# Tongdongq/darwin-gpu

Measured on AMD Instinct MI355X. Metric: GACT GCUPS (DP cells/s) on ~10 kb PacBio-shape reads, higher is better.
Workload: dtype int16x2 (packed); 1 GPU; ecoli10x_self_overlap; tile_size=320, tile_overlap=120, scoring=+1/-1/-1/-1, reads=4642, bases=48503677, candidates=65766, tiles=2185214, parallelism=candidates dealt round-robin over 1 GPU(s), slots_in_flight=4, passes_in_this_process=127, arch=gfx950:sramecc+:xnack-

## Files before the change

darwin-gpu_amd/csrc/gact_coop.hpp:

```cpp
#pragma once

#include "gact_lin.hpp"

namespace gact {

constexpr int kCoopBanks = 2;
constexpr int kCoopJobs = (kBlockThreads / 64) * 8 * kCoopBanks;
static_assert(kCoopJobs == 64, "a walking wave serves every job of its block, one per lane");
constexpr int kCoopCacheStride = 36;

struct CoopJob {
    uint32_t ws_off;
    int R, Q;
    int k0;
    int v0;
    int band_lim;
    uint32_t where;
    int pad_;
};
struct CoopDone { int ref_steps, query_steps, dv, redo; };

template <class L> constexpr size_t coop_bank_words() { return (size_t)L::G::kMaxFlush * L::kWalkQuads * kWsRow * 4; }
template <class L> __host__ constexpr size_t coop_ws_words(int blocks) { return (size_t)blocks * (kBlockThreads / 64) * kCoopBanks * coop_bank_words<L>(); }

// ... 60 lines not shown
        const uint32_t rw = stage[seg + (rp >> 4)], qw = stage[seg + kSeg + (qp >> 4)];
        rcode = __builtin_amdgcn_ubfe(rw, ((uint32_t)rp & 15u) << 1, 2u);
        qcode = __builtin_amdgcn_ubfe(qw, ((uint32_t)qp & 15u) << 1, 2u);
    };
#ifdef GACT_STAMPS
    unsigned long long n_trips = 0, n_lane_trips = 0;
#endif
    while (__any(go)) {
        if (go) {
            tb_refill_oct<CW, QN, ROW>(ws_all, ws_off, scratch, l, c, k, rg);
            off0 = 4 * (-8 * rg.fbase[0] - 4 * rg.qbase0);
            off1 = 4 * (16 - 8 * rg.fbase[1] - 4 * (QN - 2));
            cur = fetch(l, c, k);
            bases();
        }
#pragma unroll 1
        for (int m = 0; m < 8; m++) {
            if (!__any(go)) break;
#ifdef GACT_STAMPS
            n_trips++; n_lane_trips += (unsigned long long)__builtin_popcountll(__ballot(go));
#endif
            if (go) {
                const bool diag = cur == kM;
                const int sub = rcode == qcode ? v_match : v_mism;
                v -= diag ? sub : v_gap;
                nis -= cur != kD;
                njs -= cur != kI;
                const int p = imax(p0 + njs, 0);
                l = (int)(__umul24((uint32_t)p, kMagic) >> 16);
                c = p + __mul24(l, -CW);
                k = imax(kA + l + nis, 0);
                if (m == 7) {
                    redo = redo | ((band_lim >= 0) & ((unsigned)(nis - njs + band_lim) > (unsigned)(2 * band_lim)));
                } else {
                    cur = fetch(l, c, k);
                    bases();
                }
                go = !((diag && v == 0) || nis <= nlim_i || njs <= nlim_j || redo);
            }
        }
    }
    if (active) {
        done[lane].ref_steps = -nis; done[lane].query_steps = -njs; done[lane].dv = v0 - v; done[lane].redo = redo ? 1 : 0;
        __builtin_amdgcn_fence(__ATOMIC_RELEASE, "workgroup");
        __hip_atomic_store(&jstate[lane], st0 + 2u, __ATOMIC_RELAXED, __HIP_MEMORY_SCOPE_WORKGROUP);
    }
#ifdef GACT_STAMPS
    {
        const unsigned long long n_jobs = (unsigned long long)__builtin_popcountll(__ballot(active));
        if (lane == 0) { atomicAdd(&g_coop_counts[0], 1ull); atomicAdd(&g_coop_counts[1], n_trips); atomicAdd(&g_coop_counts[2], n_lane_trips);
                         atomicAdd(&g_coop_counts[3], n_jobs); }
    }
#endif
}

template <class L, bool TWO_SETS = false>
__global__ __launch_bounds__(kBlockThreads, 3) void extend_coop_kernel(
    KParams kp, P16Consts kc, SeqSetDev refs, SeqSetDev qfwd, SeqSetDev qrc,
    int same_file, gact_overlap *__restrict__ out, ChainQueues cq,
    uint32_t *__restrict__ ws_all)
{
    using G = typename L::G;
    constexpr int LANES = L::kLanes;
    static_assert(LANES == kGroup && L::kWalkFmt == 3 && L::kEndAligned, "the split linear-gap layout");
    constexpr int kGroupsOfWave = 64 / LANES;
    constexpr int kGroupsPerBlock = (kBlockThreads / 64) * kGroupsOfWave;
    constexpr int kStageWords = StageGeom<L::kSlotsPerLane, LANES>::kWords;
    constexpr int kSeg = StageGeom<L::kSlotsPerLane, LANES>::kSeg;
    static_assert(((kGroupsPerBlock * kCoopBanks * kStageWords) >> 15) == 0, "stage index fits CoopJob::where");
    constexpr int kRefBytes = (G::kRefBytes + 15) & ~15;
    __shared__ __attribute__((aligned(16))) uint8_t lds[kGroupsPerBlock * kRefBytes];
    __shared__ ChainState chain_lds[kGroupsPerBlock][kCoopBanks][kSlots];
    __shared__ __attribute__((aligned(16))) uint32_t stage_lds[kGroupsPerBlock][kCoopBanks][kStageWords];
    __shared__ __attribute__((aligned(16))) CoopJob jobs[kCoopJobs];
    __shared__ CoopDone done[kCoopJobs];
    __shared__ uint32_t jstate[kCoopJobs];
    __shared__ __attribute__((aligned(16))) uint32_t cache_lds[kCoopJobs * kCoopCacheStride];
    __shared__ int bank_lds[kGroupsPerBlock][kCoopBanks][6];
    __shared__ uint32_t walk_lock;

    uint32_t *const lin_lut = LinLutLds<L::kLutWords>::get();
    for (int n = threadIdx.x; n < kCoopJobs; n += kBlockThreads) jstate[n] = 0;
    if (threadIdx.x == 0) walk_lock = 0;
    lin_lut_fill(lin_lut, kc, (int)threadIdx.x);
    __syncthreads();

    const int wave_in_block = threadIdx.x >> 6;
    WaveCtx w;
    {
        const int lane = threadIdx.x & 63;
        w.gl = lane & (LANES - 1);
        w.g = lane / LANES;
        w.slot = (blockIdx.x * (kBlockThreads / 64) + wave_in_block) * kGroupsOfWave + w.g;
        w.n_slots = gridDim.x * (kBlockThreads / 64) * kGroupsOfWave;
    }
    const int group_in_block = wave_in_block * kGroupsOfWave + w.g;
    uint8_t *ref8 = lds + group_in_block * kRefBytes;
    uint8_t *q8 = ref8;
    const uint16_t *ref16_lane = reinterpret_cast<const uint16_t *>(ref8) + (L::kRow0 - 1 - w.gl);
    uint32_t *ws_wave = ws_all + (size_t)(blockIdx.x * (kBlockThreads / 64) + wave_in_block) * (kCoopBanks * coop_bank_words<L>());
    const int job_base = (group_in_block * kSlots + (w.gl & 1)) * kCoopBanks;

    for (int b = 0; b < kCoopBanks; b++)
        if (w.gl < kSlots) { chain_lds[group_in_block][b][w.gl].phase = 2; chain_lds[group_in_block][b][w.gl].cand = -1; }
    if (w.gl == 0) {
        int *bt = &bank_lds[group_in_block][0][0];
        for (int n = 0; n < kCoopBanks * 6; n++) bt[n] = 0;
    }
    wave_sync();
    bool exhausted = false;
    int my_bucket = 0;
    int bucket_first = 0;
    if (cq.leave_longest > 0) {
        int acc = 0;
        while (bucket_first < kBuckets && (acc += cq.bucket_count[bucket_first]) <= cq.leave_longest) bucket_first++;
        if (bucket_first >= kBuckets) bucket_first = 0;
    }
    bool second_set = false;
    constexpr bool one_set = !TWO_SETS;
    int idle_polls = 0;
    int rank_turn = 0, rank_cached = 0;
    int bank = 0;
    __builtin_amdgcn_s_setprio(3);
#ifdef GACT_STAMPS
    unsigned long long stamp_acc[8] = {0, 0, 0, 0, 0, 0, 0, 0};
    const unsigned long long tl_start = __builtin_amdgcn_s_memrealtime();
    const unsigned long long tl_cyc0 = __builtin_amdgcn_s_memtime();
    unsigned long long tl_empty = 0;
#endif

    for (;;) {
        ChainState *st = chain_lds[group_in_block][bank];
        GACT_STAMP(t_w0);
        const int *bk = &bank_lds[group_in_block][bank][0];
        const uint32_t want = (uint32_t)__builtin_amdgcn_readfirstlane(bk[4]);
        if (want != 0) {
            const int sv_R[kSlots] = {bk[0], bk[2]}, sv_Q[kSlots] = {bk[1], bk[3]};
            const bool mine = w.gl < kSlots && ((w.gl & 1) ? sv_R[1] : sv_R[0]) > 0;
            const int my_job = job_base + bank;
            const unsigned long long wd0 = __builtin_amdgcn_s_memrealtime();
            for (;;) {
                const uint32_t s = mine ? __hip_atomic_load(&jstate[my_job], __ATOMIC_RELAXED, __HIP_MEMORY_SCOPE_WORKGROUP) : want;
                if (__all(s == want)) break;
                if (__any(mine && (s & 3u) == 1u)) {
                    uint32_t got = 1;
                    if ((threadIdx.x & 63) == 0) got = atomicCAS(&walk_lock, 0u, 1u);
                    got = (uint32_t)__builtin_amdgcn_readfirstlane((int)got);
                    if (got == 0) {
                        __builtin_amdgcn_fence(__ATOMIC_ACQUIRE, "workgroup");
                        coop_walk_batch<L>(kp, ws_all, jobs, jstate, done, &stage_lds[0][0][0], cache_lds);
                        __builtin_amdgcn_fence(__ATOMIC_RELEASE, "workgroup");
                        if ((threadIdx.x & 63) == 0) __hip_atomic_store(&walk_lock, 0u, __ATOMIC_RELAXED, __HIP_MEMORY_SCOPE_WORKGROUP);
                        continue;
                    }
                }
                __builtin_amdgcn_s_sleep(4);
                if (__builtin_amdgcn_s_memrealtime() - wd0 > 200000000ull) {
                    if ((threadIdx.x & 63) == 0) atomicOr(cq.band_redos, 1 << 30);
                    break;
                }
            }
            __builtin_amdgcn_fence(__ATOMIC_ACQUIRE, "workgroup");
            int ref_steps = 0, query_steps = 0, nst = 0, redo = 0;
            ScoreWalk wk;
            wk.score = 0; wk.pend_gap = 0; wk.open_flag = 0; wk.have_left = 0; wk.left_first_gap = 0;
            if (mine) {
                const CoopDone d = done[my_job];
// ... 202 lines not shown
```

darwin-gpu_amd/csrc/gact_engine.hip:

```cpp
#include <hip/hip_runtime.h>
#include <rccl/rccl.h>

#include <cerrno>
#include <dlfcn.h>
#include <fcntl.h>
#include <unistd.h>

#include <algorithm>
#include <atomic>
#include <chrono>
#include <condition_variable>
#include <cstdarg>
#include <cstdio>
#include <cstring>
#include <deque>
#include <memory>
#include <mutex>
#include <string>
#include <thread>
#include <vector>

#include "gact_hip.h"
#include "gact_kernels.hpp"
#include "gact_chain_kernel.hpp"
// ... 279 lines not shown
    {"force_wide", "GACT_HIP_FORCE_WIDE", 'c', 'k', "the wide layout (32 lanes per tile pair) for every main launch"},
    {"no_wide", "GACT_HIP_NO_WIDE", 'c', 'k', "never the wide layout"},
    {"no_tagged", "GACT_HIP_NO_TAGGED", 'c', 'k', "explicit pointer comparisons instead of tagged scores"},
    {"no_lin", "GACT_HIP_NO_LIN", 'c', 'k', "the affine passes also for linear scorings (gact_lin.hpp off)"},
    {"no_aff", "GACT_HIP_NO_AFF", 'c', 'k', "round 1's tagged affine pass instead of the drifted one (gact_aff.hpp off)"},
    {"coop", "GACT_HIP_COOP", 'l', 'k', "the split linear-gap main launch with two banks of tiles per wave and cooperative, batched traceback walks (gact_coop.hpp): 1 always, 0 never, 2 / unset where throughput bounds the launch"},
    {"roles", "GACT_HIP_ROLES", 'l', 'k', "1: the split linear-gap main launch as DP waves + walker waves (gact_roles.hpp; default 0: measured no faster, DESIGN 3.13)"},
    {"no_routing", "GACT_HIP_NO_ROUTING", 'c', 'k', "a set with a non-ACGT byte moves the whole launch onto the raw-byte kernels"},
    {"no_side_lane", "GACT_HIP_NO_SIDE_LANE", 'c', 's', "routed raw-byte launches after the 2-bit ones instead of beside them"},
    {"band", "GACT_HIP_BAND", 'c', 'k', "width of the stored pointer band in columns (default 48; 0: the whole window)"},
    {"poison_ws", "GACT_HIP_POISON_WS", 'c', 'k', "<seed>: seeded garbage over the traceback workspace before every launch (tests)"},
    {"no_overlap", "GACT_HIP_NO_OVERLAP", 'c', 's', "seed launch, then one main launch, always; live: overlap_seed"},
    {"overlap_seed", nullptr, 'l', 's', "1 / 0: ordered, overlapped seeding of large runs on an idle engine"},
    {"shared_twelfths", "GACT_HIP_SHARED_TWELFTHS", 'l', 's', "<n>: a linear-gap main launch that shares the machine and has more chains than two thirds of the resident tile slots hold takes n twelfths of the resident blocks (default 6)"},
    {"lone_lane", "GACT_HIP_LONE_LANE", 'l', 's', "<n>: a run of half as many to as many chains as there are resident tile slots, alone on the machine, runs as one block per CU of two kinds: n wide blocks for its longest chains, split blocks with the look-ahead walker on the other CUs (-n: without it); 0 (default): all wide, two blocks per CU"},
    {"overlap_big", "GACT_HIP_OVERLAP_BIG", 'l', 's', "1 / 0 (default): ... also of runs of more than four chains per resident tile slot (seed launch A takes the longest eighth, B the rest beside main launch 1; +1.3 % on pacbio50mb alone)"},
    {"no_crit_lane", "GACT_HIP_NO_CRIT_LANE", 'c', 's', "no wide launch beside the split one for runs of 1-1.5 chains per tile slot"},
    {"crit_lane_always", "GACT_HIP_CRIT_LANE_ALWAYS", 'c', 's', "... also for runs of up to four chains per tile slot"},
    {"no_shared_hint", "GACT_HIP_NO_SHARED_HINT", 'c', 's', "a launch made while another slot runs may take the wide layout"},
    {"runs_in_flight", nullptr, 'l', 's', "1: the caller keeps several runs in flight (every launch takes the throughput layout)"},
    {"no_combine", "GACT_HIP_NO_COMBINE", 'c', 's', "runs of several threads are never merged into one launch; live: combine"},
    {"combine", nullptr, 'l', 's', "1 / 0: the call combiner"},
    {"combine_window_us", "GACT_HIP_COMBINE_US", 'l', 's', "how long a leader waits for the other feeder threads (default 1000)"},
    {"sdma_copies", "GACT_HIP_SDMA_COPIES", 'c', 's', "candidate lists and records through hipMemcpyAsync instead of a copy kernel"},
    {"dsoft_temp_cap", "GACT_HIP_DSOFT_TEMP_CAP", 'c', 'k', "initial size of the device filter's candidate staging area (tests: forces the regrow path)"},
    {"rccl_lib", "GACT_HIP_RCCL_LIB", 'c', 's', "<file>: the RCCL library gact_hip_comm_create loads"},
    {"path_budget_mb", "GACT_HIP_PATH_BUDGET_MB", 'c', 's', "<n>: MiB of column buffers a path run (gact_hip_candidates_paths) takes at most; larger selections run in chunks (default 1024)"},
    {"no_aff_seed", "GACT_HIP_NO_AFF_SEED", 'c', 'd', "round 1's packed seed pass for affine scorings"},
    {"lane_blocks", "GACT_HIP_LANE_BLOCKS", 'c', 'd', "<n>: blocks of the critical lane"},
    {"lane_small", "GACT_HIP_LANE_SMALL", 'c', 'd', "<f>: the lane also instead of the all-wide launch, for runs of at least f/2 chains per lane tile"},
    {"no_chain_prio", "GACT_HIP_NO_CHAIN_PRIO", 'c', 'd', "all DP passes at issue priority 0"},
    {"static_prio", "GACT_HIP_STATIC_PRIO", 'c', 'd', "fixed priority thresholds instead of the ranking against the longest running chain"},
    {"rank16", "GACT_HIP_RANK16", 'c', 'd', "the ranking's two thresholds in sixteenths, hi << 8 | mid (default 12, 8)"},
    {"team_when_shared", "GACT_HIP_TEAM_WHEN_SHARED", 'c', 'd', "look-ahead walker in split launches that share the machine"},
    {"wide_blocks_per_cu", "GACT_HIP_WIDE_BLOCKS_PER_CU", 'c', 'd', "<n>: resident blocks per CU of the wide launch"},
    {"band_quantum", "GACT_HIP_BAND_QUANTUM", 'c', 'd', "<1|4|8>: lanes store their band in aligned groups"},
    {"lin_blocks", "GACT_HIP_LIN_BLOCKS", 'c', 'd', "<n>: a smaller persistent grid for the one-wave-does-all split linear-gap launch"},
    {"role_blocks", "GACT_HIP_ROLE_BLOCKS", 'c', 'd', "<n>: a smaller persistent grid for the role launch"},
    {"trace", "GACT_HIP_TRACE", 'c', 'd', "every launch of a run named on stderr and waited for"},
    {"trace_upload", "GACT_HIP_TRACE_UPLOAD", 'c', 'd', "stamps inside candidates_upload / _fetch on stderr"},
};
static const char *opt_env(const char *name)
{
    for (const OptionDef &o : kOptions)
        if (!strcmp(o.name, name)) {
#ifndef GACT_EXPERIMENTS
            if (o.klass == 'd') return nullptr;
#endif
            return o.env ? getenv(o.env) : nullptr;
        }
    fprintf(stderr, "[gact_hip] internal: switch '%s' is not in the option table\n", name);
    abort();
}

struct RunReq {
    int slot, first, n, rc_from, same_file;
    int status = 0;
    bool launched = false;
    std::string err;
};
struct Combiner {
    std::mutex mu;
    std::condition_variable cv;
    std::vector<RunReq *> pending;
    bool leader = false;
    bool enabled = true;
    int window_us = 1000;
    int next_merge = 0;
    int n_merge = 0;
    long merged_launches = 0, merged_runs = 0, rejoins = 0;
    std::vector<std::shared_ptr<LaunchStats>> stats_pool;
};

struct gact_hip_engine {
    gact_hip_params params;
    gact::KParams kp{};
    int C = 20;
    int big_cb = 0;
    int big_blocks = 0;
    bool p16 = false;
    bool split = false;
    bool tagged = false;
    bool lin = false;
    bool aff = false;
    bool aff_seed = true;
    int wide = 0;
    int wide_blocks_per_cu = 0;
    bool crit_lane = true;
    int lane_blocks = 0;
    bool lane_small = false;
    int lane_small_factor = 3;
    bool crit_lane_always = false;
    bool kernel_copies = true;
    bool shared_hint = true;
    std::atomic<bool> caller_keeps_runs_in_flight{false};
    bool team_when_shared = false;
    bool overlap_seed = true;
    bool side_lane = true;
    bool route_other = true;
    bool chain_prio = true;
    bool static_prio = false;
    uint32_t poison = 0;
    int rank16 = (12 << 8) | 8;
    bool seed16 = false;
    int seed_grid_blocks = 0;
    int seed_lin_grid_blocks = 0;
    int lin_grid_blocks = 0;
    bool roles = false;
    int role_grid_blocks = 0;
    int shared_twelfths = 6;
    int lone_lane = 0;
    bool overlap_big = false;
    int coop = 0;
    int64_t path_budget = 1024ll << 20;
    int aff_grid_blocks = 0;
    int wide_lin_grid_blocks = 0;
    gact::P16Consts kc;
    hipDeviceProp_t prop;
    int grid_blocks = 0;
    int blocks_per_cu = 0;
    size_t ws_words_total = 0;
    SeqSet sets[GACT_NUM_SETS];
    std::vector<Slot> slots;
    int n_user = 0;
    Combiner cb;
    std::mutex upload_mu;
    int64_t sets_epoch = 0;
    DsoftState dsoft;
    std::mutex dsoft_mu;
    int64_t ref_epoch = 0;
    Pileup pileup;
};

namespace {

int set_device(gact_hip_engine *e)
{
    HIP_TRY(hipSetDevice(e->params.device_id));
    return 0;
}

int check_slot(gact_hip_engine *e, int slot)
{
    if (!e) return fail(GACT_HIP_EINVAL, "engine is NULL");
    if (slot < 0 || slot >= e->n_user)
        return fail(GACT_HIP_EINVAL, "slot %d out of range [0,%d)", slot, e->n_user);
    return 0;
}

void note_call(gact_hip_engine *e, int slot)
{
    if (!e->cb.enabled || e->n_user < 2) return;
    std::lock_guard<std::mutex> lk(e->cb.mu);
    Slot &sl = e->slots[slot];
    sl.last_thread = std::this_thread::get_id();
    sl.last_call = std::chrono::steady_clock::now();
}

constexpr int kMoreCount = 8 + 2 * gact::kBuckets + gact::kEpochs, kMorePop = kMoreCount + gact::kBuckets;
constexpr int kOrderHist = kMorePop + gact::kBuckets, kOrderCursor = kOrderHist + gact::kBuckets;
constexpr int kCounterInts = kOrderCursor + gact::kBuckets;

int poison_ws(gact_hip_engine *e, Slot &sl, uint32_t salt);

struct StreamPool {
    std::mutex mu;
// ... 238 lines not shown
    const Lane own = main_lane(e, sl);
    const int blocks = std::max(1, std::min((n + 3) / 4, e->big_blocks));
    auto k = e->big_cb == 16 ? gact::big_extend_kernel<16> : gact::big_extend_kernel<32>;
    hipLaunchKernelGGL(k, dim3(blocks), dim3(gact::kBlockThreads), 0, sl.stream, e->kp, rs.dev(true), qf.dev_or(true, rs),
                       qr.dev_or(true, rs), sl.cands.p, first, n, rc_from, same_file, sl.overlaps.p, queues(own, sl),
                       reinterpret_cast<uint8_t *>(sl.d_ws));
    HIP_TRY(hipGetLastError());
    return 0;
}

gact_policy::Caps policy_caps(const gact_hip_engine *e)
{
    gact_policy::Caps c;
    c.C = e->C; c.p16 = e->p16; c.seed16 = e->seed16; c.lin = e->lin; c.aff = e->aff; c.aff_seed = e->aff_seed; c.split = e->split; c.tagged = e->tagged;
    c.mismatch_below_extend = e->params.mismatch < e->params.gap_extend;
    c.shared_twelfths = e->shared_twelfths; c.lone_lane = e->lone_lane; c.overlap_big = e->overlap_big; c.roles = e->roles; c.coop = (e->lin && e->split && e->C == 20) ? e->coop : -1; c.overlap_seed = e->overlap_seed; c.crit_lane = e->crit_lane; c.crit_lane_always = e->crit_lane_always;
    c.lane_small = e->lane_small; c.lane_small_factor = e->lane_small_factor; c.lane_blocks = e->lane_blocks; c.team_when_shared = e->team_when_shared;
    c.wide = e->wide; c.wide_blocks_per_cu = e->wide_blocks_per_cu; c.cus = e->prop.multiProcessorCount;
    c.grid_blocks = e->grid_blocks; c.seed_grid_blocks = e->seed_grid_blocks; c.seed_lin_grid_blocks = e->seed_lin_grid_blocks;
    c.lin_grid_blocks = e->lin_grid_blocks; c.aff_grid_blocks = e->aff_grid_blocks; c.wide_lin_grid_blocks = e->wide_lin_grid_blocks;
    c.role_grid_blocks = e->role_grid_blocks; c.role_dp_waves = gact::kRoleDp;
    c.ws_words_per_tile = (size_t)e->kp.ws_words;
    c.role_ws_words_per_block = gact::role_ws_words<gact::SplitLayoutLin<7, 13>>(1);
    c.coop_ws_words_per_block = gact::coop_ws_words<gact::SplitLayoutLin<7, 13>>(1);
    return c;
}

template <int C>
int launch_extend(gact_hip_engine *e, Slot &sl, int first, int n, int rc_from, int same_file, int strands = -1)
{
    const SeqSet &rs = e->sets[GACT_SET_REF];
    const SeqSet &qf = e->sets[GACT_SET_QUERY], &qr = e->sets[GACT_SET_QUERY_RC];
    const bool need_f = strands >= 0 ? (strands & 1) != 0 : first < rc_from, need_r = strands >= 0 ? (strands & 2) != 0 : first + n > rc_from;
    const bool any_other = rs.has_other || (need_f && qf.has_other) || (need_r && qr.has_other);
    const bool mixed = any_other && e->p16 && e->route_other;
    gact::KParams kp = e->kp;
    const int64_t longest = std::min(rs.max_len, std::max(need_f ? qf.max_len : 0, need_r ? qr.max_len : 0));
    const bool static_prio = e->static_prio;
    kp.prio_bases[0] = !e->chain_prio ? 0x7fffffff : static_prio ? (int32_t)std::min<int64_t>(longest / 3, 0x7fffffff) : 0;
    const int rank16 = e->rank16;
    kp.prio_bases[1] = !e->chain_prio ? 0x7fffffff : static_prio ? (int32_t)std::min<int64_t>(2 * longest / 3, 0x7fffffff) : rank16;
    sl.two_phase = e->p16;
    sl.routed_raw = 0;
    sl.overlapped = false;
    sl.lane = false;
    sl.roles = 0;
    bool shared_machine = e->caller_keeps_runs_in_flight.load(std::memory_order_relaxed);
    if (e->shared_hint && !shared_machine)
        for (const Slot &other : e->slots)
            if (&other != &sl && other.timed && other.ev1 && hipEventQuery(other.ev1) == hipErrorNotReady) { shared_machine = true; break; }
    (void)hipGetLastError();

    static const bool trace = opt_env("trace") != nullptr;
    auto traced = [&](const Lane &ln, const char *what, int blocks, int count) -> int {
        if (!trace) return 0;
        fprintf(stderr, "[gact_hip] %s: %d blocks, %d candidates ... ", what, blocks, count);
        fflush(stderr);
        HIP_TRY(hipStreamSynchronize(ln.stream));
        int dbg[8];
        HIP_TRY(hipMemcpy(dbg, ln.d_counter, sizeof dbg, hipMemcpyDeviceToHost));
        fprintf(stderr, "done (popped %d)\n", dbg[0]);
        return 0;
    };
    auto run_pass = [&](const Lane &ln, bool raw, const int *list, const int *list_count, int count, bool first_pass, bool second_set = false) -> int {
        namespace pol = gact_policy;
        pol::Inputs in;
        in.count = count; in.raw = raw; in.listed = list != nullptr; in.second_set = second_set; in.shared_machine = shared_machine;
        in.own_lane = ln.stream == sl.stream; in.trace = trace; in.poison = e->poison != 0; in.lane_max_blocks = ln.max_blocks;
        const pol::Plan plan = pol::plan_pass(policy_caps(e), in);
        const gact::SeqSetDev d_rs = rs.dev(raw), d_qf = qf.dev_or(raw, rs), d_qr = qr.dev_or(raw, rs);
        gact::ChainQueues cq = second_set ? second_queues(ln, sl) : queues(ln, sl);
        cq.list = list; cq.list_count = list_count;
        if (trace) {
            fprintf(stderr, "[gact_hip] pass raw=%d listed=%d side=%d count=%d first=%d n=%d rc_from=%d plan=%s\n", (int)raw, list != nullptr,
                    ln.stream != sl.stream, count, first, n, rc_from, pol::describe(plan).c_str());
            fprintf(stderr, "[gact_hip]   ws %p + %zu MiB, counter %p, cands %p (%zu), overlaps %p, live %p (%zu), states %p (%zu x %zu B)\n", (void *)ln.d_ws,
                    ln.ws_words * 4 >> 20, (void *)ln.d_counter, (void *)sl.cands.p, sl.cands.cap, (void *)sl.overlaps.p, (void *)ln.live,
                    ln.live_cap, (void *)sl.chain_states.p, sl.chain_states.cap, sizeof(gact::ChainState));
            fprintf(stderr, "[gact_hip]   ref raw %p packed %p offsets %p (%lld bases), query %p %p, rc %p %p\n", (void *)rs.d_raw, (void *)rs.d_packed,
                    (void *)rs.d_offsets, (long long)rs.total, (void *)qf.d_raw, (void *)qf.d_packed, (void *)qr.d_raw, (void *)qr.d_packed);
        }
        using gact::extend_p16_kernel;
        using RolesL = gact::SplitLayoutLin<7, 13>;
        auto launch_main = [&](pol::MainK k, bool two_sets, int blocks, hipStream_t stream, const gact::ChainQueues &q, uint32_t *ws) -> int {
            using M = pol::MainK;
            const dim3 g((unsigned)blocks), b256(gact::kBlockThreads), brole(gact::kRoleThreads);
#define GACT_LAUNCH_MAIN(KERNEL, BLOCK) hipLaunchKernelGGL(KERNEL, g, BLOCK, 0, stream, kp, e->kc, d_rs, d_qf, d_qr, same_file, sl.overlaps.p, q, ws)
            if constexpr (C == 20) {
                switch (k) {
                case M::RolesLin: if (two_sets) GACT_LAUNCH_MAIN((gact::extend_roles_kernel<RolesL, true>), brole); else GACT_LAUNCH_MAIN((gact::extend_roles_kernel<RolesL, false>), brole); break;
                case M::CoopLin: if (two_sets) GACT_LAUNCH_MAIN((gact::extend_coop_kernel<RolesL, true>), b256); else GACT_LAUNCH_MAIN((gact::extend_coop_kernel<RolesL, false>), b256); break;
                case M::SplitLin: if (two_sets) GACT_LAUNCH_MAIN((extend_p16_kernel<gact::SplitLayoutLin<7, 13>, false, true>), b256); else GACT_LAUNCH_MAIN((extend_p16_kernel<gact::SplitLayoutLin<7, 13>, false>), b256); break;
                case M::SplitLinTeam: GACT_LAUNCH_MAIN((extend_p16_kernel<gact::SplitLayoutLinTeam<7, 13>, false>), b256); break;
                case M::WideLin: if (two_sets) GACT_LAUNCH_MAIN((extend_p16_kernel<gact::WideLayoutLin, false, true>), b256); else GACT_LAUNCH_MAIN((extend_p16_kernel<gact::WideLayoutLin, false>), b256); break;
                case M::SplitAffNeg: GACT_LAUNCH_MAIN((extend_p16_kernel<gact::SplitLayoutAff<7, 13, true>, false>), b256); break;
                case M::SplitAff: GACT_LAUNCH_MAIN((extend_p16_kernel<gact::SplitLayoutAff<7, 13, false>, false>), b256); break;
                default: break;
                }
            }
            switch (k) {
            case M::WideTaggedRaw: GACT_LAUNCH_MAIN((extend_p16_kernel<gact::WideLayoutTagged, true>), b256); break;
            case M::WideTagged: GACT_LAUNCH_MAIN((extend_p16_kernel<gact::WideLayoutTagged, false>), b256); break;
            case M::WideRaw: GACT_LAUNCH_MAIN((extend_p16_kernel<gact::WideLayout, true>), b256); break;
            case M::Wide: GACT_LAUNCH_MAIN((extend_p16_kernel<gact::WideLayout, false>), b256); break;
            case M::SplitTaggedRaw: GACT_LAUNCH_MAIN((extend_p16_kernel<gact::SplitLayout<7, 13, true>, true>), b256); break;
            case M::SplitTagged: GACT_LAUNCH_MAIN((extend_p16_kernel<gact::SplitLayout<7, 13, true>, false>), b256); break;
            case M::SplitRaw: GACT_LAUNCH_MAIN((extend_p16_kernel<gact::SplitLayout<7, 13>, true>), b256); break;
            case M::Split: GACT_LAUNCH_MAIN((extend_p16_kernel<gact::SplitLayout<7, 13>, false>), b256); break;
            case M::UniformTaggedRaw: GACT_LAUNCH_MAIN((extend_p16_kernel<gact::UniformLayout<C, gact::kGroup, true>, true>), b256); break;
            case M::UniformTagged: GACT_LAUNCH_MAIN((extend_p16_kernel<gact::UniformLayout<C, gact::kGroup, true>, false>), b256); break;
            case M::UniformRaw: GACT_LAUNCH_MAIN((extend_p16_kernel<gact::UniformLayout<C>, true>), b256); break;
            case M::Uniform: GACT_LAUNCH_MAIN((extend_p16_kernel<gact::UniformLayout<C>, false>), b256); break;
            default: break;
            }
#undef GACT_LAUNCH_MAIN
            HIP_TRY(hipGetLastError());
            return 0;
        };
        auto launch_seed = [&](pol::SeedK k, int blocks, hipStream_t stream, const gact::ChainQueues &q, uint32_t *ws) -> int {
            using S = pol::SeedK;
            const dim3 g((unsigned)blocks), b256(gact::kBlockThreads);
#define GACT_LAUNCH_SEED(KERNEL) hipLaunchKernelGGL(KERNEL, g, b256, 0, stream, kp, e->kc, d_rs, d_qf, d_qr, sl.cands.p, first, n, rc_from, same_file, sl.overlaps.p, q, ws)
            if constexpr (C == 20) {
                switch (k) {
                case S::P16Lin: GACT_LAUNCH_SEED((gact::seed_p16_kernel<C, false, 1>)); break;
                case S::P16Aff: GACT_LAUNCH_SEED((gact::seed_p16_kernel<C, false, 2>)); break;
                case S::P16AffNeg: GACT_LAUNCH_SEED((gact::seed_p16_kernel<C, false, 3>)); break;
                default: break;
                }
            }
            switch (k) {
            case S::P16Raw: GACT_LAUNCH_SEED((gact::seed_p16_kernel<C, true>)); break;
            case S::P16: GACT_LAUNCH_SEED((gact::seed_p16_kernel<C, false>)); break;
            case S::Int32:
                hipLaunchKernelGGL((gact::chain_kernel<C, gact::SeedSink>), g, b256, 0, stream, kp, d_rs, d_qf, d_qr, sl.cands.p, n, rc_from,
                                   same_file, sl.overlaps.p, q, gact::SeedSink{first, e->p16 ? 1 : 0}, ws);
                break;
            default: break;
            }
#undef GACT_LAUNCH_SEED
            HIP_TRY(hipGetLastError());
            return 0;
        };
        int rc = 0;
        if (plan.seq == pol::Seq::Overlapped) {
            if ((rc = ensure_aux_stream(sl))) return rc;
            const int ob = std::max(1, std::min((count + 255) / 256, 1024));
            hipLaunchKernelGGL(gact::order_hist_kernel, dim3(ob), dim3(256), 0, ln.stream, sl.cands.p, first, count, rc_from, d_rs.offsets,
                               d_qf.offsets, d_qr.offsets, kp.early, ln.d_counter + kOrderHist);
            hipLaunchKernelGGL(gact::order_scatter_kernel, dim3(ob), dim3(256), 0, ln.stream, sl.cands.p, first, count, rc_from,
                               d_rs.offsets, d_qf.offsets, d_qr.offsets, kp.early, ln.d_counter + kOrderHist,
                               ln.d_counter + kOrderCursor, sl.order.p);
            HIP_TRY(hipGetLastError());
            const int nA = plan.nA;
            gact::ChainQueues qa = queues(ln, sl);
            qa.list = sl.order.p; qa.list_n = nA;
            if ((rc = launch_seed(plan.seed, plan.seed_blocks, ln.stream, qa, ln.d_ws))) return rc;
            if (first_pass) HIP_TRY(hipEventRecord(sl.ev_mid, ln.stream));
            HIP_TRY(hipEventRecord(sl.aux_ev_a, ln.stream));
            HIP_TRY(hipStreamWaitEvent(sl.aux_stream, sl.aux_ev_a, 0));
            gact::ChainQueues qb = second_queues(ln, sl);
            qb.list = sl.order.p + nA; qb.list_n = count - nA;
            if (count > nA && (rc = launch_seed(plan.seed, plan.seedB_blocks, sl.aux_stream, qb, ln.d_ws + plan.ws_split))) return rc;
            HIP_TRY(hipMemsetAsync(ln.d_counter + 7, 0xff, sizeof(int), sl.aux_stream));
            gact::ChainQueues q2 = queues(ln, sl);
            {
                const gact::ChainQueues s2 = second_queues(ln, sl);
                q2.more_flag = ln.d_counter + 7;
                q2.more_count = s2.bucket_count; q2.more_pop = s2.bucket_pop; q2.more_live = s2.live;
            }
            if (count > nA && (rc = launch_main(plan.lane ? pol::MainK::WideLin : plan.main, true, plan.main2_blocks, sl.aux_stream, q2, ln.d_ws + plan.ws_split))) return rc;
            HIP_TRY(hipEventRecord(sl.aux_ev_b, sl.aux_stream));
// ... 36 lines not shown
                       rc_from, o_rs.other, need_f ? o_qf.other : nullptr, need_r ? o_qr.other : nullptr, sl.deferred.p, sl.d_counter + 4);
    HIP_TRY(hipGetLastError());
    int routed[2] = {0, 0};
    const bool host_counts = strands < 0 && !sl.h_cands.empty() && (size_t)first + (size_t)n <= sl.h_cands.size() &&
                             (!rs.has_other || (int32_t)rs.h_other.size() == rs.n) && (!need_f || !qf.has_other || (int32_t)qf.h_other.size() == qf.n) &&
                             (!need_r || !qr.has_other || (int32_t)qr.h_other.size() == qr.n);
    if (host_counts) {
        const int64_t key[4] = {first, n, rc_from, e->sets_epoch};
        if (memcmp(key, sl.routed_key, sizeof key)) {
            int dirty = 0;
            for (int k = first; k < first + n; k++) {
                const gact_candidate &c = sl.h_cands[(size_t)k];
                const SeqSet &qs = k >= rc_from ? qr : qf;
                dirty += ((rs.has_other && rs.h_other[(size_t)c.ref_id]) || (qs.has_other && qs.h_other[(size_t)c.query_id])) ? 1 : 0;
            }
            memcpy(sl.routed_key, key, sizeof key);
            sl.routed_host[0] = n - dirty; sl.routed_host[1] = dirty;
        }
        routed[0] = sl.routed_host[0]; routed[1] = sl.routed_host[1];
    } else {
        HIP_TRY(hipMemcpyAsync(routed, sl.d_counter + 4, sizeof routed, hipMemcpyDeviceToHost, sl.stream));
        HIP_TRY(hipStreamSynchronize(sl.stream));
    }
    sl.routed_raw = routed[1];
    int rc = 0;
    const int side_cap = std::max(1, e->prop.multiProcessorCount / 2);
    const int raw_blocks = ((routed[1] + 2 * gact::kGroupsPerWave - 1) / (2 * gact::kGroupsPerWave) + 3) / 4;
    if (routed[0] > 0 && routed[1] > 0 && e->side_lane && raw_blocks <= side_cap) {
        Lane side;
        if ((rc = side_lane(e, sl, routed[1], std::max(raw_blocks, std::min(side_cap, 16)), &side))) return rc;
        HIP_TRY(hipEventRecord(sl.side_go, sl.stream));
        HIP_TRY(hipStreamWaitEvent(side.stream, sl.side_go, 0));
        HIP_TRY(hipMemsetAsync(side.d_counter, 0, kCounterInts * sizeof(int), side.stream));
        HIP_TRY(hipEventRecord(sl.side_go, side.stream));
        HIP_TRY(hipStreamWaitEvent(sl.stream, sl.side_go, 0));
        if ((rc = poison_lane(e, side, 0x1b873593u))) return rc;
        if ((rc = run_pass(side, true, sl.deferred.p + n, sl.d_counter + 5, routed[1], false))) return rc;
        HIP_TRY(hipEventRecord(sl.side_done, side.stream));
        sl.side_used = true;
        rc = run_pass(own, false, sl.deferred.p, sl.d_counter + 4, routed[0], true);
        if (hipStreamWaitEvent(sl.stream, sl.side_done, 0) != hipSuccess && !rc) return fail(GACT_HIP_EDEVICE, "hipStreamWaitEvent failed");
        return rc;
    }
    if (routed[0] > 0 && (rc = run_pass(own, false, sl.deferred.p, sl.d_counter + 4, routed[0], true))) return rc;
    if (routed[1] == 0) return 0;
    if (routed[0] > 0) { int prc = poison_ws(e, sl, 0x1b873593u); if (prc) return prc; }
    return run_pass(own, true, sl.deferred.p + n, sl.d_counter + 5, routed[1], routed[0] == 0, routed[0] > 0);
}

template <int C> int occupancy_blocks(int *out)
{
    int a = 0, b = 0;
    HIP_TRY(hipOccupancyMaxActiveBlocksPerMultiprocessor(&a, gact::chain_kernel<C, gact::SeedSink>, gact::kBlockThreads, 0));
    HIP_TRY(hipOccupancyMaxActiveBlocksPerMultiprocessor(&b, gact::align_tiles_kernel<C>, gact::kBlockThreads, 0));
    int m = std::min(a, b);
    for (int v = 0; v < 14; v++) {
        int c = m;
        if (v == 12 || v == 13) continue;
        auto k = v == 13 ? gact::extend_p16_kernel<gact::WideLayoutLin, false>
               : v == 0 ? gact::extend_p16_kernel<gact::UniformLayout<C>, true>
               : v == 1 ? gact::extend_p16_kernel<gact::UniformLayout<C>, false>
               : v == 2 ? gact::extend_p16_kernel<gact::SplitLayout<7, 13>, true>
               : v == 3 ? gact::extend_p16_kernel<gact::SplitLayout<7, 13>, false>
               : v == 4 ? gact::extend_p16_kernel<gact::WideLayout, true>
               : v == 5 ? gact::extend_p16_kernel<gact::WideLayout, false>
               : v == 6 ? gact::extend_p16_kernel<gact::SplitLayout<7, 13, true>, true>
               : v == 7 ? gact::extend_p16_kernel<gact::SplitLayout<7, 13, true>, false>
               : v == 8 ? gact::extend_p16_kernel<gact::WideLayoutTagged, true>
               : v == 9 ? gact::extend_p16_kernel<gact::WideLayoutTagged, false>
               : v == 10 ? gact::extend_p16_kernel<gact::UniformLayout<C, gact::kGroup, true>, true>
                         : gact::extend_p16_kernel<gact::UniformLayout<C, gact::kGroup, true>, false>;
        HIP_TRY(hipOccupancyMaxActiveBlocksPerMultiprocessor(&c, k, gact::kBlockThreads, 0));
        m = std::min(m, c);
    }
    *out = std::max(1, m);
    return 0;
}

int lin_occupancy_blocks(int *out)
{
    int a = 0;
    HIP_TRY(hipOccupancyMaxActiveBlocksPerMultiprocessor(&a, gact::extend_p16_kernel<gact::SplitLayoutLin<7, 13>, false>,
                                                         gact::kBlockThreads, 0));
    int b = a;
    HIP_TRY(hipOccupancyMaxActiveBlocksPerMultiprocessor(&b, gact::extend_p16_kernel<gact::SplitLayoutLinTeam<7, 13>, false>,
                                                         gact::kBlockThreads, 0));
    *out = std::max(1, std::min(a, b));
    return 0;
}

template <int C> int seed_occupancy_blocks(int *out, int *out_lin)
{
    int a = 0, b = 0;
    HIP_TRY(hipOccupancyMaxActiveBlocksPerMultiprocessor(&a, gact::seed_p16_kernel<C, true>, gact::kBlockThreads, 0));
    HIP_TRY(hipOccupancyMaxActiveBlocksPerMultiprocessor(&b, gact::seed_p16_kernel<C, false>, gact::kBlockThreads, 0));
    int c = b;
    if constexpr (C == 20) {
        HIP_TRY(hipOccupancyMaxActiveBlocksPerMultiprocessor(&c, gact::seed_p16_kernel<C, false, 1>, gact::kBlockThreads, 0));
        int d = b;
        HIP_TRY(hipOccupancyMaxActiveBlocksPerMultiprocessor(&d, gact::seed_p16_kernel<C, false, 3>, gact::kBlockThreads, 0));
        b = std::min(b, d);
    }
    *out = std::max(1, std::min(a, b));
    *out_lin = std::max(1, c);
    return 0;
}

int validate_tiles(gact_hip_engine *e, const SeqSet &rs, const SeqSet &qf, const SeqSet &qr, int n,
                   const gact_tile *tiles)
{
    const int T = e->params.tile_size;
    for (int t = 0; t < n; t++) {
        const gact_tile &d = tiles[t];
        if (d.ref_len < 0) continue;
        const SeqSet &qs = (d.query_set == GACT_SET_QUERY_RC) ? qr : qf;
        if (d.query_set != GACT_SET_QUERY && d.query_set != GACT_SET_QUERY_RC)
            return fail(GACT_HIP_EINVAL, "tile %d: query_set %d", t, d.query_set);
        if (d.ref_len > T || d.query_len > T || d.query_len < 0)
            return fail(GACT_HIP_ERANGE, "tile %d: length %d x %d exceeds tile_size %d", t, d.ref_len,
                        d.query_len, T);
        if (d.ref_id < 0 || d.ref_id >= rs.n || d.query_id < 0 || d.query_id >= qs.n)
            return fail(GACT_HIP_ERANGE, "tile %d: sequence id out of range", t);
        const int64_t rl = rs.h_offsets[d.ref_id + 1] - rs.h_offsets[d.ref_id];
        const int64_t ql = qs.h_offsets[d.query_id + 1] - qs.h_offsets[d.query_id];
        if (d.ref_off < 0 || d.ref_off + (int64_t)d.ref_len > rl || d.query_off < 0 ||
            d.query_off + (int64_t)d.query_len > ql)
            return fail(GACT_HIP_ERANGE, "tile %d: slice outside its sequence", t);
    }
    return 0;
}

int run_tiles(gact_hip_engine *e, Slot &sl, const SeqSet &rs, const SeqSet &qf, const SeqSet &qr, int32_t n,
              const gact_tile *tiles, gact_tile_result *results, uint8_t *states, int32_t states_stride)
{
    if (n == 0) return 0;
    if (!rs.d_raw) return fail(GACT_HIP_EINVAL, "align_tiles: the reference read set has not been uploaded");
    if (sl.tiles.reserve(n) || sl.results.reserve(n) || sl.states.reserve((size_t)n * states_stride))
        return fail(GACT_HIP_ENOMEM, "device allocation failed");
    HIP_TRY(hipMemcpyAsync(sl.tiles.p, tiles, (size_t)n * sizeof(gact_tile), hipMemcpyHostToDevice, sl.stream));
    HIP_TRY(hipMemsetAsync(sl.results.p, 0, (size_t)n * sizeof(gact_tile_result), sl.stream));
    { int prc = poison_ws(e, sl, 0x2545f491u); if (prc) return prc; }
    HIP_TRY(hipEventRecord(sl.ev0, sl.stream));
    sl.forget_times();
    int rc = e->big_cb ? launch_big_tiles(e, sl, rs, qf, qr, n, states_stride)
           : (e->C == 20) ? launch_tiles<20>(e, sl, rs, qf, qr, n, states_stride)
                          : launch_tiles<32>(e, sl, rs, qf, qr, n, states_stride);
    if (rc) return rc;
    HIP_TRY(hipEventRecord(sl.ev1, sl.stream));
    sl.timed = true;
    HIP_TRY(hipMemcpyAsync(results, sl.results.p, (size_t)n * sizeof(gact_tile_result), hipMemcpyDeviceToHost,
                           sl.stream));
    HIP_TRY(hipMemcpyAsync(states, sl.states.p, (size_t)n * states_stride, hipMemcpyDeviceToHost, sl.stream));
    HIP_TRY(hipStreamSynchronize(sl.stream));
    return 0;
}

}

extern "C" {

const char *gact_hip_last_error(void) { return g_err.c_str(); }

static bool derive_kernel_flags(gact_hip_engine *e)
{
    const gact_hip_params *p = &e->params;
    e->C = (p->tile_size <= 20 * gact::kGroup) ? 20 : 32;
    const bool big = p->tile_size > 32 * gact::kGroup;
    if (big) e->big_cb = p->tile_size <= gact::BigGeom<16>::kTileMax ? 16 : 32;
    e->kp.tile_size = p->tile_size;
    e->kp.early = p->tile_size - p->tile_overlap;
    e->kp.match = p->match; e->kp.mismatch = p->mismatch;
    e->kp.open = p->gap_open; e->kp.ext = p->gap_extend;
    e->kp.thr = p->first_tile_score_threshold;
    e->kp.ws_words = (e->C == 20) ? gact::Geometry<20>::kWsWords : gact::Geometry<32>::kWsWords;
    e->p16 = !big && gact::p16_scoring_ok(p->tile_size, p->match, p->mismatch, p->gap_open, p->gap_extend) &&
             opt_env("force_int32") == nullptr;
    e->split = e->p16 && e->C == 20 && e->kp.early <= gact::GeometrySplit<7, 13>::W2 &&
               opt_env("force_uniform") == nullptr;
    e->tagged = e->p16 && gact::p16_tagged_ok(p->tile_size, p->match, p->mismatch, p->gap_open, p->gap_extend) &&
                opt_env("no_tagged") == nullptr;
    e->lin = e->tagged && gact::p16_lin_ok(p->tile_size, p->match, p->mismatch, p->gap_open, p->gap_extend) &&
             opt_env("no_lin") == nullptr;
    e->aff = e->tagged && e->split && !e->lin && gact::p16_aff_ok(p->tile_size, p->match, p->mismatch, p->gap_open, p->gap_extend) &&
             opt_env("no_aff") == nullptr;
    e->aff_seed = opt_env("no_aff_seed") == nullptr;
    e->kernel_copies = opt_env("sdma_copies") == nullptr;
    e->crit_lane = opt_env("no_crit_lane") == nullptr;
    e->crit_lane_always = opt_env("crit_lane_always") != nullptr;
    if (const char *v = opt_env("lane_blocks")) e->lane_blocks = std::max(0, atoi(v));
    if (const char *v = opt_env("lane_small")) { e->lane_small = atoi(v) > 0; e->lane_small_factor = std::max(1, atoi(v)); }
    e->seed16 = e->p16 && gact::p16_argmax_ok(p->tile_size, p->match) && opt_env("force_int32_seed") == nullptr;
    e->chain_prio = opt_env("no_chain_prio") == nullptr;
    e->route_other = opt_env("no_routing") == nullptr;
    e->side_lane = opt_env("no_side_lane") == nullptr;
    e->shared_hint = opt_env("no_shared_hint") == nullptr;
    e->overlap_seed = opt_env("no_overlap") == nullptr;
    e->roles = opt_env("roles") != nullptr && atoi(opt_env("roles")) != 0;
    if (const char *v = opt_env("overlap_big")) e->overlap_big = atoi(v) != 0;
    if (const char *v = opt_env("shared_twelfths")) e->shared_twelfths = std::max(1, std::min(atoi(v), 12));
    if (const char *v = opt_env("lone_lane")) e->lone_lane = std::max(-255, std::min(atoi(v), 255));
    if (const char *v = opt_env("coop")) e->coop = atoi(v) == 1 ? 1 : atoi(v) == 0 ? -1 : 0;
    e->team_when_shared = opt_env("team_when_shared") != nullptr;
    e->static_prio = opt_env("static_prio") != nullptr;
    if (const char *v = opt_env("rank16")) e->rank16 = atoi(v);
    if (const char *v = opt_env("poison_ws")) e->poison = (uint32_t)strtoul(v, nullptr, 0) | 0x80000000u;
    e->wide = opt_env("force_wide") ? 1 : opt_env("no_wide") ? -1 : 0;
    if (const char *v = opt_env("wide_blocks_per_cu")) e->wide_blocks_per_cu = atoi(v);
    return big;
}

int gact_hip_create(const gact_hip_params *p, gact_hip_engine **out)
{
    if (!p || !out) return fail(GACT_HIP_EINVAL, "create: NULL argument");
    *out = nullptr;
    if (p->tile_size < 1 || p->tile_size > GACT_HIP_MAX_TILE)
        return fail(GACT_HIP_EINVAL, "tile_size %d not in [1,%d]", p->tile_size, GACT_HIP_MAX_TILE);
    if (p->tile_overlap < 0 || p->tile_overlap >= p->tile_size)
        return fail(GACT_HIP_EINVAL, "tile_overlap %d must be in [0, tile_size)", p->tile_overlap);
    if (p->mismatch > 0 || p->gap_open > 0 || p->gap_extend > 0)
        return fail(GACT_HIP_EINVAL, "scoring: mismatch, gap_open and gap_extend must be <= 0");
    if (p->match < 0 || (int64_t)p->match * p->tile_size > (1 << 28) ||
        p->mismatch < -(1 << 20) || p->gap_open < -(1 << 20) || p->gap_extend < -(1 << 20))
        return fail(GACT_HIP_EINVAL, "scoring: values out of the int32-safe range");
    if (p->first_tile_score_threshold < 1)
        return fail(GACT_HIP_EINVAL, "first_tile_score_threshold must be >= 1 (the reference loops forever otherwise, gact.cpp:82)");
    if (p->n_slots < 1 || p->n_slots > 256) return fail(GACT_HIP_EINVAL, "n_slots %d not in [1,256]", p->n_slots);

    int ndev = 0;
    if (hipGetDeviceCount(&ndev) != hipSuccess || ndev <= 0)
        return fail(GACT_HIP_EDEVICE, "no HIP device visible: this engine has no CPU fallback");
    if (p->device_id < 0 || p->device_id >= ndev)
        return fail(GACT_HIP_EINVAL, "device_id %d not in [0,%d)", p->device_id, ndev);

#ifdef GACT_EXPERIMENTS
    fprintf(stderr, "[gact_hip] built with -DGACT_EXPERIMENTS: timing experiments may be compiled in, results are NOT to be trusted\n");
#endif
    gact_hip_engine *e = new gact_hip_engine();
    e->params = *p;
    int rc = set_device(e);
    if (rc) { delete e; return rc; }
    if (hipGetDeviceProperties(&e->prop, p->device_id) != hipSuccess) {
        delete e;
        return fail(GACT_HIP_EDEVICE, "hipGetDeviceProperties failed");
    }
    const bool big = derive_kernel_flags(e);
    e->kp.prio_bases[0] = e->kp.prio_bases[1] = 0x7fffffff;
    e->kp.band = gact::kLinBandDefault;
    if (const char *v = opt_env("band")) {
        const int b = atoi(v);
        e->kp.band = b <= 0 ? 0 : std::max(b, gact::kLinBandMin);
    }
    if (e->kp.band >= e->kp.early) e->kp.band = 0;
    {
        int q = gact::kLinBandQuantum;
        if (const char *v = opt_env("band_quantum")) q = atoi(v);
        q = q >= 8 ? 8 : q >= 4 ? 4 : q >= 2 ? 2 : 1;
        if (e->kp.band) e->kp.band |= q << 16;
    }
    static_assert(gact::GeometrySplit<7, 13>::kWsWords <= gact::Geometry<20>::kWsWords, "workspace too small");
    e->kc.match = gact::pk2(p->match); e->kc.nd = gact::pk2(p->mismatch - p->match);
    e->kc.open = gact::pk2(p->gap_open); e->kc.ext = gact::pk2(p->gap_extend);
    e->kc.ninf = gact::pk2(gact::kNegInf16); e->kc.one = gact::pk2(1);
    e->kc.mism = gact::pk2(p->mismatch); e->kc.dsub = (uint32_t)(p->match - p->mismatch) << 24;
    e->kc.c3 = gact::pk2(3); e->kc.nmask = ~e->kc.c3; e->kc.tag1 = gact::pk2(1); e->kc.tag2 = gact::pk2(2);
    e->kc.match4 = gact::pk2(4 * p->match); e->kc.mism4 = gact::pk2(4 * p->mismatch);
    e->kc.nd4 = gact::pk2(4 * (p->mismatch - p->match));
    e->kc.open4m2 = gact::pk2(4 * p->gap_open - 2); e->kc.ext4m2 = gact::pk2(4 * p->gap_extend - 2);
    e->kc.ext4m1 = gact::pk2(4 * p->gap_extend - 1);
    e->kc.dsub4 = (uint32_t)(4 * (p->match - p->mismatch)) << 24; e->kc.floor4 = gact::pk2(-6000);
    e->kc.next = gact::pk2(-p->gap_extend); e->kc.next4 = gact::pk2(-4 * p->gap_extend);
    e->kc.ext4 = gact::pk2(4 * p->gap_extend);
    e->kc.s_mismatch = p->mismatch; e->kc.s_open = p->gap_open; e->kc.s_ext = p->gap_extend;

    rc = (e->C == 20) ? occupancy_blocks<20>(&e->blocks_per_cu) : occupancy_blocks<32>(&e->blocks_per_cu);
    if (rc) { delete e; return rc; }
    e->grid_blocks = e->blocks_per_cu * e->prop.multiProcessorCount;
    {
        int sb = 0, sbl = 0;
        rc = (e->C == 20) ? seed_occupancy_blocks<20>(&sb, &sbl) : seed_occupancy_blocks<32>(&sb, &sbl);
        if (rc) { delete e; return rc; }
        e->seed_grid_blocks = std::min(sb * e->prop.multiProcessorCount, e->grid_blocks);
        e->seed_lin_grid_blocks = std::min(sbl * e->prop.multiProcessorCount, e->grid_blocks);
    }
    e->lin_grid_blocks = e->grid_blocks;
    auto ws_words_for = [&](int blocks) { return ::ws_words_for(e, blocks); };
    if (e->lin) {
        int lb = 0;
        if ((rc = lin_occupancy_blocks(&lb))) { delete e; return rc; }
        e->lin_grid_blocks = std::max(e->grid_blocks, lb * e->prop.multiProcessorCount);
        if (const char *v = opt_env("lin_blocks")) e->lin_grid_blocks = std::max(1, std::min(atoi(v), e->lin_grid_blocks));
        int wb = 0;
        if (hipOccupancyMaxActiveBlocksPerMultiprocessor(&wb, gact::extend_p16_kernel<gact::WideLayoutLin, false>, gact::kBlockThreads, 0) !=
            hipSuccess) {
            delete e;
            return fail(GACT_HIP_EDEVICE, "hipOccupancyMaxActiveBlocksPerMultiprocessor failed");
        }
        e->wide_lin_grid_blocks = std::max(e->grid_blocks, wb * e->prop.multiProcessorCount);
        if ((ws_words_for(std::max(e->lin_grid_blocks, e->wide_lin_grid_blocks)) + 64) * sizeof(uint32_t) >= (1ull << 32)) {
            e->lin = false;
            e->lin_grid_blocks = e->grid_blocks;
        }
    }
    if (!e->lin) e->wide_lin_grid_blocks = e->grid_blocks;
    e->role_grid_blocks = 0;
    if (e->lin && e->split && e->C == 20) {
        using RL = gact::SplitLayoutLin<7, 13>;
        int rb = 0, rb2 = 0;
        if (hipOccupancyMaxActiveBlocksPerMultiprocessor(&rb, gact::extend_roles_kernel<RL, false>, gact::kRoleThreads, 0) != hipSuccess ||
            hipOccupancyMaxActiveBlocksPerMultiprocessor(&rb2, gact::extend_roles_kernel<RL, true>, gact::kRoleThreads, 0) != hipSuccess) {
            delete e;
            return fail(GACT_HIP_EDEVICE, "hipOccupancyMaxActiveBlocksPerMultiprocessor failed");
        }
        e->role_grid_blocks = std::max(1, std::min(rb, rb2)) * e->prop.multiProcessorCount;
        if (const char *v = opt_env("role_blocks")) e->role_grid_blocks = std::max(1, std::min(atoi(v), e->role_grid_blocks));
    }
    e->roles = e->roles && e->role_grid_blocks > 0;
    e->aff_grid_blocks = e->grid_blocks;
    if (e->aff) {
        int ab = 0;
        if (hipOccupancyMaxActiveBlocksPerMultiprocessor(&ab, gact::extend_p16_kernel<gact::SplitLayoutAff<7, 13, true>, false>,
                                                         gact::kBlockThreads, 0) != hipSuccess) {
            delete e;
            return fail(GACT_HIP_EDEVICE, "hipOccupancyMaxActiveBlocksPerMultiprocessor failed");
        }
        e->aff_grid_blocks = std::max(1, ab) * e->prop.multiProcessorCount;
    }
    if (p->max_blocks > 0) {
        for (int *g : {&e->grid_blocks, &e->seed_grid_blocks, &e->seed_lin_grid_blocks, &e->lin_grid_blocks, &e->wide_lin_grid_blocks, &e->aff_grid_blocks})
            *g = std::max(1, std::min(*g, (int)p->max_blocks));
        if (e->role_grid_blocks > 0) e->role_grid_blocks = std::max(1, std::min(e->role_grid_blocks, (int)p->max_blocks * 4 / (gact::kRoleDp + gact::kRoleWalk)));
    }
    e->ws_words_total = ws_words_for(std::max(std::max(e->grid_blocks, e->aff_grid_blocks), std::max(e->lin_grid_blocks, e->wide_lin_grid_blocks)));
    if (e->role_grid_blocks > 0) {
        using RL = gact::SplitLayoutLin<7, 13>;
        const int r1 = e->role_grid_blocks * 2 / 3, r2 = e->role_grid_blocks - r1;
        const size_t need = std::max(gact::role_ws_words<RL>(e->role_grid_blocks),
                                     gact::role_ws_words<RL>(r1) + std::max(gact::role_ws_words<RL>(r2), ws_words_for(e->lin_grid_blocks - e->lin_grid_blocks * 2 / 3)));
        if ((need + 64) * sizeof(uint32_t) >= (1ull << 32)) { e->roles = false; e->role_grid_blocks = 0; }
        else e->ws_words_total = std::max(e->ws_words_total, need);
    }
    if (big) {
        const size_t per_block = (gact::kBlockThreads / 64) * (e->big_cb == 16 ? gact::BigGeom<16>::kWsBytes : gact::BigGeom<32>::kWsBytes);
        e->big_blocks = (int)std::max<size_t>(1, std::min<size_t>(2 * (size_t)e->prop.multiProcessorCount, (2ull << 30) / per_block));
        if (p->max_blocks > 0) e->big_blocks = std::max(1, std::min(e->big_blocks, (int)p->max_blocks));
        e->ws_words_total = (size_t)e->big_blocks * per_block / sizeof(uint32_t);
    }
    if (const char *v = opt_env("path_budget_mb")) e->path_budget = std::max<int64_t>(1, atoll(v)) << 20;
    e->n_user = p->n_slots;
    e->cb.enabled = opt_env("no_combine") == nullptr && !big;
    if (const char *v = opt_env("combine_window_us")) e->cb.window_us = std::max(0, atoi(v));
    e->cb.n_merge = (e->cb.enabled && p->n_slots > 1) ? 2 : 0;
    e->slots.resize(p->n_slots + e->cb.n_merge);
    for (int k = 0; k < p->n_slots + (e->cb.n_merge ? 1 : 0); k++)
        if ((rc = init_slot(e, e->slots[k]))) { gact_hip_destroy(e); return rc; }
    *out = e;
    return 0;
}

void gact_hip_destroy(gact_hip_engine *e)
{
    if (!e) return;
    if (opt_env("trace") && e->cb.merged_launches)
        fprintf(stderr, "[gact_hip] combiner: %ld merged launches carried %ld runs, %ld times a group that had come apart was joined again\n", e->cb.merged_launches, e->cb.merged_runs, e->cb.rejoins);
    (void)hipSetDevice(e->params.device_id);
    for (auto &sl : e->slots) {
        if (sl.stream) (void)hipStreamSynchronize(sl.stream);
        sl.tiles.release(); sl.results.release(); sl.states.release();
        sl.cands.release(); sl.overlaps.release(); sl.live.release(); sl.chain_states.release(); sl.deferred.release();
        sl.inline_ref.release(); sl.inline_query.release();
        sl.path.release();
        sl.summary.release();
        sl.select.release();
        sl.cover.release();
        if (sl.pile_ev0) (void)hipEventDestroy(sl.pile_ev0);
        if (sl.pile_ev1) (void)hipEventDestroy(sl.pile_ev1);
        if (sl.d_counter) (void)hipFree(sl.d_counter);
        if (sl.d_flags) (void)hipFree(sl.d_flags);
        if (sl.d_ws) (void)hipFree(sl.d_ws);
        if (sl.side_stream) (void)hipStreamSynchronize(sl.side_stream);
        if (sl.aux_stream) {
            (void)hipStreamSynchronize(sl.aux_stream);
            (void)hipEventDestroy(sl.aux_ev_a); (void)hipEventDestroy(sl.aux_ev_b);
            (void)hipStreamDestroy(sl.aux_stream);
        }
        sl.order.release();
        sl.side_live.release();
        if (sl.side_counter) (void)hipFree(sl.side_counter);
        if (sl.side_ws) (void)hipFree(sl.side_ws);
        if (sl.side_done) (void)hipEventDestroy(sl.side_done);
        if (sl.side_go) (void)hipEventDestroy(sl.side_go);
        if (sl.side_stream) (void)hipStreamDestroy(sl.side_stream);
        if (sl.h_stage) (void)hipHostFree(sl.h_stage);
        if (sl.h_records) (void)hipHostFree(sl.h_records);
        if (sl.reg_out) { (void)hipHostUnregister(sl.reg_out); (void)hipGetLastError(); }
        if (sl.ev_ready) (void)hipEventDestroy(sl.ev_ready);
        if (sl.ev0) (void)hipEventDestroy(sl.ev0);
// ... 817 lines not shown
    HIP_TRY(hipEventSynchronize(sb.ev1));
    HIP_TRY(hipEventElapsedTime(&sb.stats.device_ms, sb.ev0, sb.ev1));
    sb.stats.launches = 1;
    sb.stats.scratch_bytes = (int64_t)sb.bytes;
    sb.timed = true;
    return 0;
}

int gact_hip_last_summaries_stats(gact_hip_engine *e, int slot, gact_summaries_stats *stats)
{
    int rc = check_slot(e, slot);
    if (rc) return rc;
    if (!stats) return fail(GACT_HIP_EINVAL, "last_summaries_stats: NULL argument");
    const Slot &sl = e->slots[slot];
    if (!sl.summary.timed) return fail(GACT_HIP_EINVAL, "last_summaries_stats: slot %d has made no summary run yet", slot);
    *stats = sl.summary.stats;
    return 0;
}

int gact_hip_sync(gact_hip_engine *e, int slot)
{
    int rc = check_slot(e, slot);
    if (rc) return rc;
    if ((rc = set_device(e))) return rc;
    HIP_TRY(hipStreamSynchronize(e->slots[slot].stream));
    if (e->cb.enabled && e->n_user > 1) {
        std::lock_guard<std::mutex> lk(e->cb.mu);
        e->slots[slot].in_flight = false;
    }
    return 0;
}

int gact_hip_last_kernel_ms(gact_hip_engine *e, int slot, float *ms)
{
    int rc = check_slot(e, slot);
    if (rc) return rc;
    if (!ms) return fail(GACT_HIP_EINVAL, "ms is NULL");
    if (!e->slots[slot].timed) return fail(GACT_HIP_EINVAL, "no kernel has been launched on slot %d", slot);
    if ((rc = set_device(e))) return rc;
    if (e->slots[slot].merged_into >= 0) {
        const std::shared_ptr<LaunchStats> rec = e->slots[slot].merged_stats;
        if (!rec) return fail(GACT_HIP_EINVAL, "slot %d: no statistics of its merged run", slot);
        HIP_TRY(hipEventSynchronize(rec->ev1));
        HIP_TRY(hipEventElapsedTime(ms, rec->ev0, rec->ev1));
        return 0;
    }
    Slot &sl = e->slots[slot];
    HIP_TRY(hipEventSynchronize(sl.ev1));
    HIP_TRY(hipEventElapsedTime(ms, sl.ev0, sl.ev1));
    return 0;
}

static void keep_times(Slot &sl, gact_hip_run_stats *st)
{
    if (sl.run_ms_kept) {
        st->total_ms = sl.run_ms[0]; st->seed_ms = sl.run_ms[1]; st->main_ms = sl.run_ms[2];
    } else {
        sl.run_ms[0] = st->total_ms; sl.run_ms[1] = st->seed_ms; sl.run_ms[2] = st->main_ms;
        sl.run_ms_kept = true;
    }
}

int gact_hip_last_run_stats(gact_hip_engine *e, int slot, gact_hip_run_stats *st)
{
    int rc = check_slot(e, slot);
    if (rc) return rc;
    if (!st) return fail(GACT_HIP_EINVAL, "stats is NULL");
    if (!e->slots[slot].timed) return fail(GACT_HIP_EINVAL, "no kernel has been launched on slot %d", slot);
    if ((rc = set_device(e))) return rc;
    memset(st, 0, sizeof *st);
    if (e->slots[slot].merged_into >= 0) {
        const std::shared_ptr<LaunchStats> rec = e->slots[slot].merged_stats;
        if (!rec) return fail(GACT_HIP_EINVAL, "slot %d: no statistics of its merged run", slot);
        st->merged_callers = e->slots[slot].merged_callers;
        st->overlapped_seeding = rec->overlapped ? 1 : 0;
        st->critical_lane = rec->lane ? 1 : 0;
        st->role_waves = rec->roles;
        HIP_TRY(hipEventSynchronize(rec->ev_done));
        HIP_TRY(hipEventElapsedTime(&st->total_ms, rec->ev0, rec->ev1));
        st->main_ms = st->total_ms;
        st->packed16 = rec->two_phase ? (rec->wide ? 3 : e->split ? 2 : 1) : 0;
        st->seed_packed16 = (rec->two_phase && e->seed16) ? 1 : 0;
        st->tagged_pointers = (rec->two_phase && e->tagged) ? 1 : 0;
        st->linear_gap = (rec->two_phase && rec->lin) ? 1 : (rec->two_phase && rec->aff) ? 2 : 0;
        st->raw_candidates = rec->routed_raw;
        if (rec->two_phase) {
            HIP_TRY(hipEventElapsedTime(&st->seed_ms, rec->ev0, rec->ev_mid));
            HIP_TRY(hipEventElapsedTime(&st->main_ms, rec->ev_mid, rec->ev1));
            const int *c = rec->h_counter;
            for (int b = 0; b < gact::kBuckets; b++) st->handed_off += c[8 + b] + c[kMoreCount + b];
            memcpy(&st->seed_cells, &c[2], sizeof(int64_t));
            st->band_redos = c[6];
            if (rec->side_used) {
                const int *cs = rec->h_counter + kCounterInts;
                for (int b = 0; b < gact::kBuckets; b++) st->handed_off += cs[8 + b];
                int64_t sc = 0;
                memcpy(&sc, &cs[2], sizeof(int64_t));
                st->seed_cells += sc;
            }
        }
        keep_times(e->slots[slot], st);
        return 0;
    }
    Slot &sl = e->slots[slot];
    st->merged_callers = 1;
    st->overlapped_seeding = sl.overlapped ? 1 : 0;
    st->critical_lane = sl.lane ? 1 : 0;
    st->role_waves = sl.roles;
    HIP_TRY(hipEventSynchronize(sl.ev1));
    HIP_TRY(hipEventElapsedTime(&st->total_ms, sl.ev0, sl.ev1));
    st->main_ms = st->total_ms;
    st->packed16 = sl.two_phase ? (sl.wide ? 3 : e->split ? 2 : 1) : 0;
    st->seed_packed16 = (sl.two_phase && e->seed16) ? 1 : 0;
    st->tagged_pointers = (sl.two_phase && e->tagged) ? 1 : 0;
    st->linear_gap = (sl.two_phase && sl.lin) ? 1 : (sl.two_phase && sl.aff) ? 2 : 0;
    st->raw_candidates = sl.routed_raw;
    if (sl.two_phase) {
        HIP_TRY(hipEventElapsedTime(&st->seed_ms, sl.ev0, sl.ev_mid));
        HIP_TRY(hipEventElapsedTime(&st->main_ms, sl.ev_mid, sl.ev1));
        int c[kCounterInts];
        HIP_TRY(hipMemcpy(c, sl.d_counter, sizeof c, hipMemcpyDeviceToHost));
        st->handed_off = 0;
        for (int b = 0; b < gact::kBuckets; b++) st->handed_off += c[8 + b] + c[kMoreCount + b];
        memcpy(&st->seed_cells, &c[2], sizeof(int64_t));
        st->band_redos = c[6];
        if (sl.side_used) {
            HIP_TRY(hipMemcpy(c, sl.side_counter, sizeof c, hipMemcpyDeviceToHost));
            for (int b = 0; b < gact::kBuckets; b++) st->handed_off += c[8 + b];
            int64_t sc = 0;
            memcpy(&sc, &c[2], sizeof(int64_t));
            st->seed_cells += sc;
        }
    }
    keep_times(sl, st);
    return 0;
}

int gact_hip_prepare(gact_hip_engine *e, int32_t expected_candidates)
{
    if (!e) return fail(GACT_HIP_EINVAL, "prepare: engine is NULL");
    if (expected_candidates < 0) return fail(GACT_HIP_EINVAL, "prepare: expected_candidates %d", expected_candidates);
    int rc = set_device(e);
    if (rc) return rc;
    std::lock_guard<std::mutex> lk(e->cb.mu);
    const int n_slots = e->n_user + (e->cb.n_merge ? 1 : 0);
    for (int k = 0; k < n_slots; k++) {
        Slot &sl = e->slots[k];
        if ((rc = init_slot(e, sl))) return rc;
        const size_t n = k >= e->n_user ? (size_t)expected_candidates
                                        : std::min<size_t>((size_t)expected_candidates, 2 * (size_t)expected_candidates / (size_t)e->n_user + 1024);
        if (n && reserve_candidates(sl, n)) return fail(GACT_HIP_ENOMEM, "prepare: device allocation failed (%zu candidates)", n);
        if (n && k < e->n_user) reserve_host_staging(sl, n);
        if (e->p16 && e->lin && e->split && e->C == 20) {
            if ((rc = ensure_aux_stream(sl))) return rc;
            if (!n && reserve_candidates(sl, 1024)) return fail(GACT_HIP_ENOMEM, "prepare: device allocation failed");
            const SeqSet &rs = e->sets[GACT_SET_REF];
            if (!rs.d_raw) continue;
            const gact::SeqSetDev d = rs.dev(false);
            HIP_TRY(hipMemsetAsync(sl.d_counter, 0, kCounterInts * sizeof(int), sl.stream));
            HIP_TRY(hipMemsetAsync(sl.d_counter + 7, 0xff, sizeof(int), sl.stream));
            HIP_TRY(hipStreamSynchronize(sl.stream));
            const Lane own = main_lane(e, sl);
            gact::ChainQueues q = queues(own, sl);
            q.list = sl.order.p; q.list_n = 0;
            gact::ChainQueues q2 = q;
            {
                const gact::ChainQueues s2 = second_queues(own, sl);
                q2.more_flag = sl.d_counter + 7;
                q2.more_count = s2.bucket_count; q2.more_pop = s2.bucket_pop; q2.more_live = s2.live;
            }
            for (hipStream_t st : {sl.stream, sl.aux_stream}) {
                hipLaunchKernelGGL((gact::seed_p16_kernel<20, false, 1>), dim3(1), dim3(gact::kBlockThreads), 0, st, e->kp, e->kc, d, d, d,
                                   sl.cands.p, 0, 0, 0, 0, sl.overlaps.p, q, sl.d_ws);
                hipLaunchKernelGGL((gact::extend_p16_kernel<gact::SplitLayoutLin<7, 13>, false>), dim3(1), dim3(gact::kBlockThreads), 0, st, e->kp,
                                   e->kc, d, d, d, 0, sl.overlaps.p, q, sl.d_ws);
                hipLaunchKernelGGL((gact::extend_p16_kernel<gact::SplitLayoutLin<7, 13>, false, true>), dim3(1), dim3(gact::kBlockThreads), 0, st,
                                   e->kp, e->kc, d, d, d, 0, sl.overlaps.p, q2, sl.d_ws);
                hipLaunchKernelGGL((gact::extend_coop_kernel<gact::SplitLayoutLin<7, 13>, false>), dim3(1), dim3(gact::kBlockThreads), 0, st,
                                   e->kp, e->kc, d, d, d, 0, sl.overlaps.p, q, sl.d_ws);
                hipLaunchKernelGGL((gact::extend_coop_kernel<gact::SplitLayoutLin<7, 13>, true>), dim3(1), dim3(gact::kBlockThreads), 0, st,
                                   e->kp, e->kc, d, d, d, 0, sl.overlaps.p, q2, sl.d_ws);
                if (e->role_grid_blocks > 0) {
                    hipLaunchKernelGGL((gact::extend_roles_kernel<gact::SplitLayoutLin<7, 13>, false>), dim3(1), dim3(gact::kRoleThreads), 0, st,
                                       e->kp, e->kc, d, d, d, 0, sl.overlaps.p, q, sl.d_ws);
                    hipLaunchKernelGGL((gact::extend_roles_kernel<gact::SplitLayoutLin<7, 13>, true>), dim3(1), dim3(gact::kRoleThreads), 0, st,
                                       e->kp, e->kc, d, d, d, 0, sl.overlaps.p, q2, sl.d_ws);
                }
                HIP_TRY(hipGetLastError());
            }
            HIP_TRY(hipStreamSynchronize(sl.stream));
            HIP_TRY(hipStreamSynchronize(sl.aux_stream));
        }
    }
    return 0;
}

int gact_hip_set_option(gact_hip_engine *e, const char *name, int32_t value)
{
    if (!e || !name) return fail(GACT_HIP_EINVAL, "set_option: NULL argument");
    const std::string n(name);
    if (n == "overlap_seed") e->overlap_seed = value != 0;
    else if (n == "runs_in_flight") e->caller_keeps_runs_in_flight.store(value != 0);
    else if (n == "combine") {
        std::lock_guard<std::mutex> lk(e->cb.mu);
        e->cb.enabled = value != 0 && e->cb.n_merge > 0;
    } else if (n == "combine_window_us") {
        std::lock_guard<std::mutex> lk(e->cb.mu);
        e->cb.window_us = std::max(0, (int)value);
    } else if (n == "overlap_big") {
        e->overlap_big = value != 0;
    } else if (n == "shared_twelfths") {
        e->shared_twelfths = std::max(1, std::min((int)value, 12));
    } else if (n == "lone_lane") {
        e->lone_lane = std::max(-255, std::min((int)value, 255));
    } else if (n == "coop") {
        if (value != 0 && !(e->lin && e->split && e->C == 20)) return fail(GACT_HIP_EINVAL, "set_option: this engine has no split linear-gap launch");
        e->coop = value == 1 ? 1 : value == 0 ? -1 : 0;
    } else if (n == "roles") {
        if (value != 0 && e->role_grid_blocks <= 0) return fail(GACT_HIP_EINVAL, "set_option: this engine was created without the role launch");
        e->roles = value != 0;
    } else {
        for (const OptionDef &o : kOptions)
            if (n == o.name) return fail(GACT_HIP_EINVAL, "set_option: '%s' is read once, in gact_hip_create%s%s", name, o.env ? ", from " : "", o.env ? o.env : "");
        return fail(GACT_HIP_EINVAL, "set_option: unknown option '%s'", name);
    }
    return 0;
}

int64_t gact_hip_plan_describe(const gact_hip_params *p, int32_t compute_units, int32_t count, int32_t flags, char *buf, int64_t cap)
{
    if (!p || compute_units < 1 || count < 0) return fail(GACT_HIP_EINVAL, "plan_describe: bad arguments");
    gact_hip_engine e;
    e.params = *p;
    const bool big = derive_kernel_flags(&e);
    std::string t;
    if (big) t = "{\"sequence\": \"one wave per tile (gact_big.hpp)\"}";
    else {
        e.prop.multiProcessorCount = compute_units;
        e.kp.ws_words = (e.C == 20) ? gact::Geometry<20>::kWsWords : gact::Geometry<32>::kWsWords;
        e.grid_blocks = e.lin_grid_blocks = e.wide_lin_grid_blocks = e.aff_grid_blocks = e.seed_lin_grid_blocks = 3 * compute_units;
        e.seed_grid_blocks = 2 * compute_units;
        e.role_grid_blocks = (e.lin && e.split && e.C == 20) ? compute_units : 0;
        if (flags & 4) e.roles = e.role_grid_blocks > 0;
        e.coop = (flags & 8) ? 1 : (flags & 16) ? -1 : 0;
        if (flags & 32) e.overlap_big = true;
        if (flags & 64) e.lone_lane = 48;
        gact_policy::Inputs in;
        in.count = count; in.raw = (flags & 1) != 0; in.shared_machine = (flags & 2) != 0;
        t = gact_policy::describe(gact_policy::plan_pass(policy_caps(&e), in));
    }
    if (buf && cap > 0) {
        const size_t n = std::min<size_t>((size_t)cap - 1, t.size());
        memcpy(buf, t.data(), n);
        buf[n] = 0;
    }
    return (int64_t)t.size() + 1;
}

int64_t gact_hip_options_describe(char *buf, int64_t cap)
{
    std::string t;
    for (const OptionDef &o : kOptions) {
        t += o.name; t += " | "; t += o.env ? o.env : "-"; t += " | ";
        t += o.when == 'l' ? "live (gact_hip_set_option)" : "gact_hip_create"; t += " | ";
        t += o.klass == 'k' ? "kernels" : o.klass == 's' ? "scheduling" : "diagnostic (-DGACT_EXPERIMENTS)";
        t += " | "; t += o.doc; t += "\n";
    }
    if (buf && cap > 0) {
        const size_t n = std::min<size_t>((size_t)cap - 1, t.size());
        memcpy(buf, t.data(), n);
// ... 142 lines not shown
```

darwin-gpu_amd/csrc/gact_lin.hpp:

```cpp
#pragma once

#include "gact_p16s.hpp"

namespace gact {

#ifndef GACT_LIN_MAX3
#define GACT_LIN_MAX3 1
#endif
constexpr int kLinFloor = GACT_LIN_MAX3 ? 1024 : 0;
__host__ __device__ constexpr int lin_base(int g) { return kLinFloor + 40 * (-g) + 8; }
__device__ __forceinline__ uint32_t vconst(uint32_t s)
{
    uint32_t r;
    asm volatile("s_nop 1\n\tv_mov_b32 %0, %1" : "=v"(r) : "s"(s));
    return r;
}

__host__ inline bool p16_lin_ok(int tile, int match, int mismatch, int open, int ext)
{
    const long long steps = (long long)tile + 4 * kGroup + 64 + 48;
    return open == ext && mismatch == ext && ext <= 0 && match >= 0 &&
           p16_tagged_ok(tile, match, mismatch, open, ext) &&
           4 * ((long long)match * (tile + 2) + (long long)(-ext) * steps + kLinFloor) + 3 <= 30000 && match - ext <= 63;
}

#ifndef GACT_LIN_BUILTINS
#define GACT_LIN_BUILTINS 0
#endif
typedef short LinS2 __attribute__((ext_vector_type(2)));
__device__ __forceinline__ uint32_t lin_max(uint32_t a, uint32_t b)
{
#if GACT_LIN_BUILTINS
    return __builtin_bit_cast(uint32_t, __builtin_elementwise_max(__builtin_bit_cast(LinS2, a), __builtin_bit_cast(LinS2, b)));
#else
    return pk_max(a, b);
#endif
}
__device__ __forceinline__ uint32_t lin_sub(uint32_t a, uint32_t b)
{
#if GACT_LIN_BUILTINS
    return __builtin_bit_cast(uint32_t, (LinS2)(__builtin_bit_cast(LinS2, a) - __builtin_bit_cast(LinS2, b)));
#else
    return pk_sub(a, b);
#endif
}
__device__ __forceinline__ uint32_t pk_mad4v(uint32_t a, uint32_t v_c)
{
    uint32_t r;
    asm("v_pk_mad_u16 %0, %1, 4, %2 op_sel_hi:[1,0,1]" : "=v"(r) : "v"(a), "v"(v_c));
    return r;
}
__device__ __forceinline__ uint32_t pk_max3f(uint32_t a, uint32_t b, uint32_t c)
{
    uint32_t r;
    asm("v_pk_maximum3_f16 %0, %1, %2, %3" : "=v"(r) : "v"(a), "v"(b), "v"(c));
    return r;
}
__device__ __forceinline__ uint32_t andn_or(uint32_t a, uint32_t b, uint32_t c)
{
#if GACT_LIN_BUILTINS
    return __builtin_amdgcn_bitop3_b32(a, b, c, 0xba);
#else
    uint32_t r;
    asm("v_bitop3_b32 %0, %1, %2, %3 bitop3:0xba" : "=v"(r) : "v"(a), "v"(b), "v"(c));
    return r;
#endif
}
__device__ __forceinline__ uint32_t pk_ashr2(uint32_t a)
{
#if GACT_LIN_BUILTINS
    return __builtin_bit_cast(uint32_t, (LinS2)(__builtin_bit_cast(LinS2, a) >> (short)2));
#else
    uint32_t r;
    asm("v_pk_ashrrev_i16 %0, 2, %1 op_sel_hi:[0,1]" : "=v"(r) : "v"(a));
    return r;
#endif
}


__device__ __forceinline__ uint32_t sconst_here(uint32_t lit)
{
    uint32_t r;
    asm volatile("s_mov_b32 %0, %1" : "=s"(r) : "i"(lit));
    return r;
}

template <int CW> struct LinWords {
    static constexpr int kWords = (CW + 1) / 2;
    static constexpr int kUint4 = (kWords + 3) / 4;
};
template <int NW, int LANES, class Fix>
__device__ __forceinline__ void lin_flush(const uint32_t (&acc)[2 * NW], uint4 *qA, uint4 *qB, Fix fix, const bool storeA, const bool storeB)
{
    constexpr int QD = (NW + 3) / 4;
    uint32_t wa[QD * 4], wb[QD * 4];
#pragma unroll
    for (int n = 0; n < QD * 4; n++) {
        wa[n] = n < NW ? fix(__builtin_amdgcn_perm(acc[n < NW ? 2 * n + 1 : 0], acc[n < NW ? 2 * n : 0], 0x05040100u)) : 0u;
        wb[n] = n < NW ? fix(__builtin_amdgcn_perm(acc[n < NW ? 2 * n + 1 : 0], acc[n < NW ? 2 * n : 0], 0x07060302u)) : 0u;
    }
    if (storeA) {
#pragma unroll
        for (int q = 0; q < QD; q++) qA[q * kWsRow] = make_uint4(wa[4 * q], wa[4 * q + 1], wa[4 * q + 2], wa[4 * q + 3]);
    }
    if (storeB) {
#pragma unroll
        for (int q = 0; q < QD; q++) qB[q * kWsRow] = make_uint4(wb[4 * q], wb[4 * q + 1], wb[4 * q + 2], wb[4 * q + 3]);
    }
}

template <int S> struct LinPos { static constexpr int value = S; };
constexpr int kLinTail = -1;
constexpr uint32_t kLinPairSel = 0x06020400u;
constexpr uint32_t kLinPairMask = 0x03030303u;
constexpr uint32_t kLinFlushSelA = 0x05010400u;
constexpr uint32_t kLinFlushSelB = 0x07030602u;
template <int CW>
__device__ __forceinline__ void lin_flush_groups(const uint32_t (&grp)[2 * (CW / 2)], const uint32_t odd, uint4 *qA, uint4 *qB,
                                                 const bool storeA, const bool storeB)
{
    constexpr int NP = CW / 2, NW = LinWords<CW>::kWords, QD = LinWords<CW>::kUint4;
    uint32_t wa[QD * 4], wb[QD * 4];
    const uint32_t sA = sconst_here(kLinFlushSelA), sB = sconst_here(kLinFlushSelB);
#pragma unroll
    for (int n = 0; n < QD * 4; n++) {
        wa[n] = n < NP ? __builtin_amdgcn_perm(grp[n < NP ? 2 * n : 0], grp[n < NP ? 2 * n + 1 : 0], sA)
              : n < NW ? odd & 0xffffu : 0u;
        wb[n] = n < NP ? __builtin_amdgcn_perm(grp[n < NP ? 2 * n : 0], grp[n < NP ? 2 * n + 1 : 0], sB)
              : n < NW ? odd >> 16 : 0u;
    }
    if (storeA) {
#pragma unroll
        for (int q = 0; q < QD; q++) qA[q * kWsRow] = make_uint4(wa[4 * q], wa[4 * q + 1], wa[4 * q + 2], wa[4 * q + 3]);
    }
    if (storeB) {
#pragma unroll
        for (int q = 0; q < QD; q++) qB[q * kWsRow] = make_uint4(wb[4 * q], wb[4 * q + 1], wb[4 * q + 2], wb[4 * q + 3]);
    }
}

constexpr int kLinBandDefault = 48, kLinBandMin = 24, kLinBandQuantum = 1;
struct LinBand {
    int lo[2], hi[2];
    bool full[2];
    __device__ __forceinline__ bool store(int h, int first, int last) const { return full[h] | ((last >= lo[h]) & (first <= hi[h])); }
};
__device__ __forceinline__ void lin_band_range(LinBand &b, int h, int T_end, int behind, int dj_min, int dj_max, int band, bool full)
{
    b.full[h] = full | (band <= 0);
// ... 182 lines not shown
#pragma unroll
        for (int c = 0; c < C2; c++) {
            const bool filed = blk && c >= 2 && !(c & 1);
            const uint32_t Db = Hb - dtv;
            if (filed) x &= kLinPairMask;
            GACT_SB();
            const uint32_t Hp = lin_max(U[c], Db);
            if (!blk && c > 0) acc[c - 1] = pk_shl_add4(acc[c - 1], tprev);
            if (filed) file_group(S, c, x);
            GACT_SB();
            G[C1 + c] = andn_or(Hp, c3v, c2v);
            if (!blk || c == C2 - 1) tprev = Hp & c3v;
            else if (c & 1) x = __builtin_amdgcn_perm(Hp, Hq, psel);
            else Hq = Hp;
            GACT_SB();
            Hb = G[C1 + c];
        }
        if (!blk) acc[C2 - 1] = pk_shl_add4(acc[C2 - 1], tprev);
        else odd = S ? pk_shl_add4(odd, tprev) : tprev;
        H2 = Hb;
    };
#define GACT_LIN_BLOCK8(f) do { f(LinPos<0>{}); f(LinPos<1>{}); f(LinPos<2>{}); f(LinPos<3>{}); \
                                f(LinPos<4>{}); f(LinPos<5>{}); f(LinPos<6>{}); f(LinPos<7>{}); } while (0)
#undef GACT_SB
    auto enter_tagged = [&]() {
#pragma unroll
        for (int c = C1; c < CT; c++) G[c] = pk_mad4v(G[c], c2v);
        H2 = pk_mad4v(H2, c2v);
        Hdiag2 = pk_mad4v(Hdiag2, c2v);
        Z24 = pk_mad4v(Z2, c3v);
        rb2 = row(lut_tagged, rp[-2]); rb2b = row(lut_tagged, rp[-1]);
    };

    int t = 1;
    for (const int tP = imin(LAG, imin(tB - 1, T_end)); t <= tP; t++) step_r1();
    if (t > 1) {
#pragma unroll
        for (int c = C1; c < CT; c++) G[c] = Z2;
        H2 = Z2; Hdiag2 = Z2;
        rb2 = row(lut_plain, rp[-2]); rb2b = row(lut_plain, rp[-1]);
    }
    const int tU = imin(tB - 1, T_end);
    for (; t + 1 <= tU; t += 2) { step(); step(); }
    if (t <= tU) { step(); t++; }
    const bool tagged = t <= T_end;
    if (tagged) enter_tagged();
    uint4 *qA = reinterpret_cast<uint4 *>(wsA) + gl;
    uint4 *qB = reinterpret_cast<uint4 *>(wsB) + gl;
    LinBand bd;
    {
        const int q1 = (band >> 16) - 1, b = band & 0xffff;
        const int u_lo = kGroup - 1 - (gl & ~q1), u_hi = kGroup - 1 - (gl | q1);
        LinBand lo_, hi_;
        lin_band_range(lo_, 0, T_end, u_lo, C2 * u_lo, C2 * u_lo + C2 - 1, b, fullA);
        lin_band_range(hi_, 0, T_end, u_hi, C2 * u_hi, C2 * u_hi + C2 - 1, b, fullA);
        bd.lo[0] = bd.lo[1] = lo_.lo[0]; bd.hi[0] = bd.hi[1] = hi_.hi[0];
        bd.full[0] = fullA | (b <= 0); bd.full[1] = fullB | (b <= 0);
    }
    int k = 0;
    while (t + 7 <= T_end && t <= T_end - LAG) {
        GACT_LIN_BLOCK8(step_tagged);
        t += 8; k += 8;
        lin_flush_groups<C2>(grp, odd, qA, qB, bd.store(0, t - 8, t - 1), bd.store(1, t - 8, t - 1));
        qA += QD * kWsRow;
        qB += QD * kWsRow;
    }
    while (t + 7 <= T_end) {
        GACT_LIN_BLOCK8(step_tagged_r2);
        t += 8; k += 8;
        lin_flush_groups<C2>(grp, odd, qA, qB, bd.store(0, t - 8, t - 1), bd.store(1, t - 8, t - 1));
        qA += QD * kWsRow;
        qB += QD * kWsRow;
    }
#undef GACT_LIN_BLOCK8
    for (; t <= T_end - LAG; t++, k++) step_tagged(LinPos<kLinTail>{});
    for (; t <= T_end; t++, k++) step_tagged_r2(LinPos<kLinTail>{});
    if (k & 7) {
        const int sh = 2 * (8 - (k & 7));
        lin_flush<NW, kGroup>(acc, qA, qB, [sh](uint32_t w) { return ((w & 0xffffu) << sh & 0xffffu) | ((w >> 16) << sh << 16); },
                              bd.store(0, t - (k & 7), t - 1), bd.store(1, t - (k & 7), t - 1));
    }
    return tagged ? pk_ashr2(lin_sub(H2 | kc.c3, Z24)) : lin_sub(H2, Z2);
}

template <int C, int LANES, bool AMAX>
__device__ __forceinline__ uint32_t dp_pass_lin(const P16Consts &kc, const int gl,
                                                const uint16_t *__restrict__ ref16,
                                                const uint32_t (&qb)[C],
                                                const int T_end, const int tB,
                                                uint32_t *__restrict__ wsA, uint32_t *__restrict__ wsB,
                                                const int cqA, const int cqB, const int (*RQ)[2], P16Best *pb,
                                                const int col_from, const int band, const int QA, const int QB,
                                                const bool fullA, const bool fullB)
{
    constexpr int NW = LinWords<C>::kWords, QD = LinWords<C>::kUint4;
    const bool store = AMAX || gl * C + C >= col_from;
    LinBand bd;
    {
        const int q1 = AMAX ? 0 : (band >> 16) - 1, b = AMAX ? 0 : band & 0xffff;
        const int g_lo = gl & ~q1, g_hi = gl | q1;
        LinBand lo_, hi_;
        lin_band_range(lo_, 0, T_end, (imax(QA, 1) - 1) / C - g_lo, QA - g_lo * C - C, QA - g_lo * C - 1, b, fullA);
        lin_band_range(lo_, 1, T_end, (imax(QB, 1) - 1) / C - g_lo, QB - g_lo * C - C, QB - g_lo * C - 1, b, fullB);
        lin_band_range(hi_, 0, T_end, (imax(QA, 1) - 1) / C - g_hi, QA - g_hi * C - C, QA - g_hi * C - 1, b, fullA);
        lin_band_range(hi_, 1, T_end, (imax(QB, 1) - 1) / C - g_hi, QB - g_hi * C - C, QB - g_hi * C - 1, b, fullB);
        bd = lo_;
        bd.hi[0] = hi_.hi[0] < 0 ? (lo_.hi[0] < 0 ? lo_.hi[0] : T_end) : hi_.hi[0];
        bd.hi[1] = hi_.hi[1] < 0 ? (lo_.hi[1] < 0 ? lo_.hi[1] : T_end) : hi_.hi[1];
    }
    static_assert(!AMAX || LANES == kGroup, "first tiles run on the 16-lane layout");
    const int g = (int)(int16_t)(kc.ext & 0xffffu);
    const uint32_t gv = vconst(kc.next), g4v = vconst(kc.next4), c3v = vconst(kc.c3), onev = vconst(kc.one),
                   dtv = vconst(kc.next4 + kc.tag1),
                   c2v = vconst(kc.tag2), lut1v = vconst(0x01010101u);
    uint32_t Z = pk2(lin_base(g) + gl * g);
    uint32_t G[C];
    uint32_t acc[2 * NW];
#pragma unroll
    for (int c = 0; c < C; c++) G[c] = Z;
#pragma unroll
    for (int c = 0; c < 2 * NW; c++) acc[c] = 0;
    uint32_t G_last = Z, Hdiag = Z;

    uint32_t bk[AMAX ? C : 1];
    int lane_best[2] = {-1, -1};
    uint32_t col_x0 = 0;
    int t_first = 0, rows[2] = {0, 0};
    if (AMAX) {
#pragma unroll
        for (int c = 0; c < C; c++) bk[c] = 0xffffffffu;
        const int ncA = imin(imax(RQ[0][1] - gl * C, 0), C), ncB = imin(imax(RQ[1][1] - gl * C, 0), C);
        col_x0 = ((uint32_t)(-ncA) & 0xffffu) | ((uint32_t)(-ncB) << 16);
        t_first = gl + 1;
        rows[0] = RQ[0][0]; rows[1] = RQ[1][0];
    }

    auto lut = [&](uint32_t amount) { return kc.dsub >> (amount & 31u); };
    auto lut4 = [&](uint32_t amount) { return kc.dsub4 >> (amount & 31u); };
    uint32_t lutA = 0, lutB = 0;
    { const uint32_t w = ref16[1]; lutA = lut(w & 0xffu); lutB = lut(w >> 8); }

    auto shr1 = [](uint32_t v, uint32_t old) {
        return (uint32_t)(LANES == 32 ? dpp_shr1_32((int)v, (int)old) : dpp_row_shr1((int)v, (int)old));
    };

#define GACT_SB() __builtin_amdgcn_sched_barrier(0)
    auto upper_all = [&](uint32_t (&U)[C], const bool tag2, const uint32_t Zr) {
        uint32_t P[C];
#pragma unroll
        for (int c = 0; c < C; c++) P[c] = __builtin_amdgcn_perm(lutB, lutA, qb[c]);
        GACT_SB();
#pragma unroll
        for (int c = 0; c < C; c++) U[c] = (c == 0 ? Hdiag : G[c - 1]) + P[c];
        (void)tag2;
        GACT_SB();
        if (GACT_LIN_MAX3) {
#pragma unroll
            for (int c = 0; c < C; c++) U[c] = pk_max3f(U[c], Zr, G[c]);
        } else {
#pragma unroll
            for (int c = 0; c < C; c++) U[c] = lin_max(U[c], Zr);
            GACT_SB();
#pragma unroll
            for (int c = 0; c < C; c++) U[c] = lin_max(U[c], G[c]);
        }
        GACT_SB();
// ... 87 lines not shown
    const bool tagged = t <= T_end;
    if (tagged) enter_tagged();
    uint4 *qA = reinterpret_cast<uint4 *>(wsA) + gl;
    uint4 *qB = reinterpret_cast<uint4 *>(wsB) + gl;
    int k = 0;
    while (t + 7 <= T_end) {
        for (int s8 = 0; s8 < 8; s8++, t++) step_tagged(t);
        k += 8;
        lin_flush<NW, LANES>(acc, qA, qB, [](uint32_t w) { return w; }, store && bd.store(0, t - 8, t - 1), store && bd.store(1, t - 8, t - 1));
        qA += QD * kWsRow;
        qB += QD * kWsRow;
        if (AMAX) fold(k - 8);
    }
    for (; t <= T_end; t++, k++) step_tagged(t);
    if (AMAX) {
        if (k & 7) fold(k & ~7);
#pragma unroll
        for (int h = 0; h < 2; h++) {
            const int rec = lane_best[h];
            int best = 0, bi = 0, bj = 0;
            if (rec >= 0) {
                best = rec >> 15;
                bi = tB + ((rec >> 5) & 1023) - gl;
                bj = gl * C + (rec & 31) + 1;
            }
#pragma unroll
            for (int mm = 1; mm < kGroup; mm <<= 1) {
                const int ob = __shfl_xor(best, mm, kGroup);
                const int oi = __shfl_xor(bi, mm, kGroup);
                const int oj = __shfl_xor(bj, mm, kGroup);
                const bool take = (ob > best) | ((ob == best) & ((oi > bi) | ((oi == bi) & (oj > bj))));
                best = take ? ob : best;
                bi = take ? oi : bi;
                bj = take ? oj : bj;
            }
            pb->best[h] = best; pb->bi[h] = bi; pb->bj[h] = bj;
        }
    }
    if (k & 7) {
        const int sh = 2 * (8 - (k & 7));
        lin_flush<NW, LANES>(acc, qA, qB, [sh](uint32_t w) { return ((w & 0xffffu) << sh & 0xffffu) | ((w >> 16) << sh << 16); },
                             store && bd.store(0, t - (k & 7), t - 1), store && bd.store(1, t - (k & 7), t - 1));
    }
    if (AMAX) return 0;
    uint32_t ga = G[0], gb = G[0];
#pragma unroll
    for (int c = 1; c < C; c++) { ga = (c == cqA) ? G[c] : ga; gb = (c == cqB) ? G[c] : gb; }
    const uint32_t pick = __builtin_amdgcn_perm(gb, ga, 0x07060100u);
    return tagged ? pk_ashr2(lin_sub(pick | kc.c3, Z4)) : lin_sub(pick, Z);
}

struct WideLayoutLin : UniformLayout<10, 32, true> {
    static constexpr int kWalkFmt = 3, kWalkQuads = LinWords<10>::kUint4;
#ifndef GACT_WALK_SPAN
#define GACT_WALK_SPAN 16
#endif
    static constexpr int kWalkSpan = GACT_WALK_SPAN;
#ifndef GACT_WIDE_LIN_BLOCKS
#define GACT_WIDE_LIN_BLOCKS 3
#endif
    static constexpr int kBlocksPerCu = GACT_WIDE_LIN_BLOCKS;
    static constexpr bool kEndAligned = true;
    template <bool RAW>
    __device__ static uint32_t pass(const P16Consts &kc, int gl, const uint16_t *ref16, const uint32_t (&qb)[10], int T_end,
                                    int tB, uint32_t *wsA, uint32_t *wsB, const PairTile &pt)
    {
        static_assert(!RAW, "the linear-gap pass reads 2-bit sets");
        return dp_pass_lin<10, 32, false>(kc, gl, ref16, qb, T_end, tB, wsA, wsB, (imax(pt.Q[0], 1) - 1) % 10,
                                          (imax(pt.Q[1], 1) - 1) % 10, nullptr, nullptr, pt.col_from, pt.band, pt.Q[0], pt.Q[1],
                                          pt.full[0], pt.full[1]);
    }
    __device__ static int fin_lane(int Q) { return (imax(Q, 1) - 1) / 10; }
};

#ifndef GACT_LIN_BLOCKS_PER_CU
#define GACT_LIN_BLOCKS_PER_CU 3
#endif
template <int C1, int C2> struct SplitLayoutLin : SplitLayout<C1, C2, true> {
    static constexpr int kBlocksPerCu = GACT_LIN_BLOCKS_PER_CU;
    static constexpr int kWalkFmt = 3, kWalkQuads = LinWords<C2>::kUint4;
    static constexpr int kWalkSpan = GACT_WALK_SPAN;
    static constexpr bool kEndAligned = true;
    static constexpr int kLutWords = kLinLutWords;
    using Base = SplitLayout<C1, C2, true>;
    template <bool RAW>
    __device__ static void load(const SeqSetDev &rs, const SeqSetDev &qf, const SeqSetDev &qr,
                                const PairTile &pt, int gl, uint8_t *ref8, uint8_t *q8, uint32_t (&qb)[C1 + C2], uint32_t *stage)
    {
        static_assert(!RAW, "the linear-gap pass reads 2-bit sets");
        load_pair_packed<C1 + C2, kGroup, typename Base::Cols, true, kLinPadRow>(rs, qf, qr, pt, gl, ref8, Base::G::kRefBytes, Base::G::kRow0, q8,
                                                                                 Base::G::kTileMax, qb, stage, typename Base::Cols{});
    }
    template <bool RAW>
    __device__ static uint32_t pass(const P16Consts &kc, int gl, const uint16_t *ref16, const uint32_t (&qb)[C1 + C2],
                                    int T_end, int tB, uint32_t *wsA, uint32_t *wsB, const PairTile &pt)
    {
        static_assert(!RAW, "the linear-gap pass reads 2-bit sets");
        return dp_pass_lin_split<C1, C2>(kc, gl, ref16, qb, T_end, tB, wsA, wsB, pt.band, pt.full[0], pt.full[1], pt.lut);
    }
    __device__ static int fin_lane(int Q) { (void)Q; return kGroup - 1; }
};

template <int C1, int C2> struct SplitLayoutLinTeam : SplitLayoutLin<C1, C2> {
    static constexpr bool kTeamWalk = true;
};

}
```

darwin-gpu_amd/csrc/gact_p16.hpp:

```cpp
#pragma once

#include <type_traits>

#include "gact_chain.hpp"
#include "gact_kernels.hpp"

namespace gact {

#ifdef GACT_STAMPS
__device__ unsigned long long g_stamps[8];
__device__ unsigned long long g_stamps2[8];
__device__ unsigned long long g_timeline[4 * 4096];
__device__ unsigned long long g_wave_cycles[4096];
__device__ unsigned long long g_coop_counts[4];
#define GACT_STAMP(var) unsigned long long var = __builtin_amdgcn_s_memtime()
#define GACT_ACC(slot, t0, t1) stamp_acc[slot] += (t1) - (t0)
#else
#define GACT_STAMP(var)
#define GACT_ACC(slot, t0, t1)
#endif

#ifndef GACT_SEED_WALK_TEAM
#define GACT_SEED_WALK_TEAM 1
#endif
// ... 356 lines not shown
            lane_best[h] = imax(lane_best[h], m16 < 0 ? -1 : rec);
        }
    };

    int t = 1;
    for (; t < tB && t <= T_end; t++) step(t, std::false_type{});
    if (TAG) enter_tagged();
    uint4 *qA = reinterpret_cast<uint4 *>(wsA) + gl;
    uint4 *qB = reinterpret_cast<uint4 *>(wsB) + gl;
    int k = 0;
    for (; t <= T_end; t++, k++) {
        if (TAG) step_tagged(t); else step(t, std::true_type{});
        if ((k & 7) == 7) {
#pragma unroll
            for (int q = 0; q < QD; q++) {
                qA[q * kWsRow] = make_uint4(wordA(accO[4 * q], accF[4 * q]), wordA(accO[4 * q + 1], accF[4 * q + 1]),
                                            wordA(accO[4 * q + 2], accF[4 * q + 2]), wordA(accO[4 * q + 3], accF[4 * q + 3]));
                qB[q * kWsRow] = make_uint4(wordB(accO[4 * q], accF[4 * q]), wordB(accO[4 * q + 1], accF[4 * q + 1]),
                                           wordB(accO[4 * q + 2], accF[4 * q + 2]), wordB(accO[4 * q + 3], accF[4 * q + 3]));
            }
            qA += QD * kWsRow;
            qB += QD * kWsRow;
            if (AMAX) fold(k - 7);
        }
    }
    if (AMAX) {
        if (k & 7) fold(k & ~7);
#pragma unroll
        for (int h = 0; h < 2; h++) {
            const int rec = lane_best[h];
            int best = 0, bi = 0, bj = 0;
            if (rec >= 0) {
                best = rec >> 15;
                bi = tB + ((rec >> 5) & 1023) - gl;
                bj = gl * C + (rec & 31) + 1;
            }
#pragma unroll
            for (int mm = 1; mm < kGroup; mm <<= 1) {
                const int ob = __shfl_xor(best, mm, kGroup);
                const int oi = __shfl_xor(bi, mm, kGroup);
                const int oj = __shfl_xor(bj, mm, kGroup);
                const bool take = (ob > best) | ((ob == best) & ((oi > bi) | ((oi == bi) & (oj > bj))));
                best = take ? ob : best;
                bi = take ? oi : bi;
                bj = take ? oj : bj;
            }
            pb->best[h] = best; pb->bi[h] = bi; pb->bj[h] = bj;
        }
    }
    if (k & 7) {
        const int sh = 2 * (8 - (k & 7));
        auto just = [sh](uint32_t w) { return ((w & 0xffffu) << sh & 0xffffu) | ((w >> 16) << sh << 16); };
#pragma unroll
        for (int q = 0; q < QD; q++) {
            qA[q * kWsRow] = make_uint4(just(wordA(accO[4 * q], accF[4 * q])), just(wordA(accO[4 * q + 1], accF[4 * q + 1])),
                                        just(wordA(accO[4 * q + 2], accF[4 * q + 2])), just(wordA(accO[4 * q + 3], accF[4 * q + 3])));
            qB[q * kWsRow] = make_uint4(just(wordB(accO[4 * q], accF[4 * q])), just(wordB(accO[4 * q + 1], accF[4 * q + 1])),
                                        just(wordB(accO[4 * q + 2], accF[4 * q + 2])), just(wordB(accO[4 * q + 3], accF[4 * q + 3])));
        }
    }
}

constexpr uint32_t kLutPadRow = 31, kPermZero = 0x0c;
constexpr uint32_t kLinPadRow = 32;
constexpr int kLinLutWords = 10;
struct PairTile {
    int R[kSlots], Q[kSlots], shift[kSlots];
    bool reverse[kSlots];
    int64_t rp0[kSlots], qp0[kSlots];
    int comp[kSlots];
    int col_from;
    int band;
    bool full[kSlots];
    const uint32_t *lut;
};

__device__ __forceinline__ void lin_lut_fill(uint32_t *lut, const P16Consts &kc, const int tid)
{
    if (tid < kLinLutWords) {
        const uint32_t b = 8u * ((uint32_t)tid >> 1), base = (tid & 1) ? kc.dsub4 : kc.dsub;
        lut[tid] = (b < kLinPadRow ? base >> b : 0u) + ((tid & 1) ? 0x01010101u : 0u);
    }
}
template <int N> struct LinLutLds {
    __device__ __forceinline__ static uint32_t *get() { __shared__ __attribute__((aligned(8))) uint32_t words[N]; return words; }
};
template <> struct LinLutLds<0> { __device__ __forceinline__ static uint32_t *get() { return nullptr; } };

template <class L, class = void> struct lin_lut_words { static constexpr int value = 0; };
template <class L> struct lin_lut_words<L, std::void_t<decltype(L::kLutWords)>> { static constexpr int value = L::kLutWords; };

template <int C, bool RAW, int LANES = kGroup>
__device__ __forceinline__ void load_pair(const SeqSetDev &rs, const SeqSetDev &qfwd, const SeqSetDev &qrc,
                                          const PairTile &pt, int gl, uint8_t *ref8, uint8_t *q8,
                                          uint32_t (&qb)[C])
{
    using G = GeometryP16<C, LANES>;
    GACT_STAMP(l_a);
    uint32_t *ref32 = reinterpret_cast<uint32_t *>(ref8);
    for (int k = gl; k < G::kRefBytes / 4; k += LANES) ref32[k] = RAW ? 0xffffffffu : kLutPadRow * 0x01010101u;
    wave_sync();
    GACT_STAMP(l_b);
    uint32_t rv[kSlots][C], qv[kSlots][C];
#pragma unroll
    for (int h = 0; h < kSlots; h++) {
        const SeqSetDev &qs = pt.comp[h] ? qrc : qfwd;
#pragma unroll
        for (int c = 0; c < C; c++) {
            rv[h][c] = fetch_base<RAW>(rs, slice_pos(pt.rp0[h], pt.R[h], pt.reverse[h], gl * C + c));
            qv[h][c] = fetch_base<RAW>(qs, slice_pos(pt.qp0[h], pt.Q[h], pt.reverse[h], gl * C + c));
        }
    }
#ifdef GACT_STAMPS
    { uint32_t x = 0;
#pragma unroll
      for (int h = 0; h < kSlots; h++)
#pragma unroll
        for (int c = 0; c < C; c++) x ^= rv[h][c] ^ qv[h][c];
      asm volatile("" :: "v"(x)); }
#endif
    GACT_STAMP(l_c);
#pragma unroll
    for (int c = 0; c < C; c++) qb[c] = RAW ? 0u : kPermZero * 0x01010101u;
#pragma unroll
    for (int h = 0; h < kSlots; h++) {
        const int R = pt.R[h], Q = pt.Q[h];
        uint8_t *rrow = ref8 + (LANES + pt.shift[h]) * 2 + h;
#pragma unroll
        for (int c = 0; c < C; c++) {
            const int d = gl * C + c;
            if (RAW) {
                const uint32_t qcode = (d < Q) ? qv[h][c] : kQueryPad;
                if (d < R) rrow[d * 2] = (uint8_t)rv[h][c];
                q8[h * G::kTileMax + d] = (uint8_t)qcode;
                qb[c] |= qcode << (16 * h);
            } else {
                if (d < R) rrow[d * 2] = (uint8_t)(24u - rv[h][c] * 8u);
                q8[h * G::kTileMax + d] = (uint8_t)((d < Q) ? 24u - qv[h][c] * 8u : kQueryPad);
                if (d < Q) qb[c] = (qb[c] & ~(0xffu << (16 * h))) | ((qv[h][c] + 4u * h) << (16 * h));
            }
        }
    }
#ifdef GACT_STAMPS
    asm volatile("s_waitcnt lgkmcnt(0)" ::: "memory");
    GACT_STAMP(l_d);
    if ((threadIdx.x & 63) == 0) {
        atomicAdd(&g_stamps2[0], l_b - l_a); atomicAdd(&g_stamps2[1], l_c - l_b); atomicAdd(&g_stamps2[2], l_d - l_c);
        atomicAdd(&g_stamps2[3], 1ull);
    }
#endif
}

template <int CT, int LANES> struct StageGeom {
    static constexpr int kFront = 2;
    static constexpr int kSeg = kFront + CT * LANES / 16 + 1 + 3;
    static constexpr int kWords = 4 * kSeg;
};

template <int N, int KFRONT>
__device__ __forceinline__ void cut_run(const uint32_t *seg_words, int bit0, int len, bool reverse, int d0, uint32_t (&code)[N])
{
    static_assert(N <= 32, "one 64-bit window");
    typedef __attribute__((address_space(3))) const uint32_t LdsWord;
    LdsWord *st = (LdsWord *)seg_words;
    const int lo = imax(16 * KFRONT + bit0 + (reverse ? len - d0 - N : d0), 0);
    const int wi = lo >> 4;
// ... 84 lines not shown
template <int C, int LANES = kGroup, bool TAG = false> struct UniformLayout {
    using G = GeometryP16<C, LANES>;
    static constexpr int kLanes = LANES;
    static constexpr int kSlotsPerLane = C;
    static constexpr int kWalkCols = C, kWalkQuads = G::kQuads, kWalkFmt = TAG ? 2 : 1;
    static constexpr int kRow0 = LANES;
    static constexpr bool kEndAligned = false;
    __device__ static int fin_lane(int Q) { (void)Q; return 0; }
    static constexpr int kBlocksPerCu = C <= 20 ? 3 : 1;
    __device__ static int last_step(int R, int Q) { return gact::last_step<C>(R, Q); }
    __device__ static int first_pointer_step(int R, int Q, int early) { return gact::first_pointer_step<C>(R, Q, early, false); }
    template <bool RAW>
    __device__ static void load(const SeqSetDev &rs, const SeqSetDev &qf, const SeqSetDev &qr,
                                const PairTile &pt, int gl, uint8_t *ref8, uint8_t *q8, uint32_t (&qb)[C], uint32_t *stage)
    {
        if (RAW) load_pair<C, RAW, LANES>(rs, qf, qr, pt, gl, ref8, q8, qb);
        else load_pair_packed<C, LANES>(rs, qf, qr, pt, gl, ref8, G::kRefBytes, kRow0, q8, G::kTileMax, qb, stage,
                                        UniformCols<C>{});
    }
    template <bool RAW>
    __device__ static uint32_t pass(const P16Consts &kc, int gl, const uint16_t *ref16, const uint32_t (&qb)[C], int T_end,
                                    int tB, uint32_t *wsA, uint32_t *wsB, const PairTile &)
    { dp_pass_p16<C, false, RAW, LANES, TAG>(kc, gl, ref16, qb, T_end, tB, wsA, wsB); return 0; }
    __device__ static void walk_start(int R, int Q, int tB_tile, int &l, int &c, int &k)
    { l = (Q - 1) / C; c = (Q - 1) - l * C; k = R + l - tB_tile; }
    __device__ static int tile_tB(int tB, int shift) { return tB - shift; }
};

using WideLayout = UniformLayout<10, 32>;
using WideLayoutTagged = UniformLayout<10, 32, true>;

template <class L> constexpr int walk_span()
{
    if constexpr (L::kWalkFmt == 3) return L::kWalkSpan; else return 16;
}
#ifndef GACT_WALK_TEAM
#define GACT_WALK_TEAM -1
#endif
template <class L, class = void> struct layout_team_walk : std::false_type {};
template <class L> struct layout_team_walk<L, std::enable_if_t<L::kTeamWalk>> : std::true_type {};
template <class L> constexpr bool walk_by_team()
{
    if constexpr (L::kWalkFmt != 3) return false;
    else if (GACT_WALK_TEAM >= 0) return GACT_WALK_TEAM != 0;
    else return L::kLanes == 32 || layout_team_walk<L>::value;
}
template <class L, bool TEAM> constexpr int walk_scratch_words()
{
    if constexpr (TEAM) return LaRegion<L::kWalkCols, L::kWalkQuads, walk_span<L>()>::kWords; else return kTbScratchWords;
}

template <class L, bool RAW, bool TWO_SETS = false>
__global__ __launch_bounds__(kBlockThreads, L::kBlocksPerCu) void extend_p16_kernel(
    KParams kp, P16Consts kc, SeqSetDev refs, SeqSetDev qfwd, SeqSetDev qrc,
    int same_file, gact_overlap *__restrict__ out, ChainQueues cq,
    uint32_t *__restrict__ ws_all)
{
    using G = typename L::G;
    constexpr int LANES = L::kLanes;
    constexpr int kGroupsOfWave = 64 / LANES;
    constexpr int kGroupsPerBlock = (kBlockThreads / 64) * kGroupsOfWave;
    __shared__ __attribute__((aligned(16))) uint8_t lds[kGroupsPerBlock * G::kGroupLds];
    __shared__ ChainState chain_lds[kGroupsPerBlock][kSlots];
    constexpr bool kTeamWalk = walk_by_team<L>();
    constexpr int kStageHalf = (StageGeom<L::kSlotsPerLane, LANES>::kWords / kSlots + 3) & ~3;
    constexpr int kScratchWords = walk_scratch_words<L, kTeamWalk>() > kStageHalf ? walk_scratch_words<L, kTeamWalk>() : kStageHalf;
    __shared__ __attribute__((aligned(16))) uint32_t tb_lds[kGroupsPerBlock][kSlots][kScratchWords];

    WaveCtx w;
    {
        const int lane = threadIdx.x & 63;
        const int wave = (blockIdx.x * blockDim.x + threadIdx.x) >> 6;
        w.gl = lane & (LANES - 1);
        w.g = lane / LANES;
        w.slot = wave * kGroupsOfWave + w.g;
        w.n_slots = ((gridDim.x * blockDim.x) >> 6) * kGroupsOfWave;
    }
    const int group_in_block = (threadIdx.x >> 6) * kGroupsOfWave + w.g;
    uint8_t *ref8 = lds + group_in_block * G::kGroupLds;
    uint8_t *q8 = ref8 + G::kRefBytes;
    const uint16_t *ref16_lane = reinterpret_cast<const uint16_t *>(ref8) + (L::kRow0 - 1 - w.gl);
    uint32_t *const lin_lut = LinLutLds<lin_lut_words<L>::value>::get();
    if constexpr (lin_lut_words<L>::value > 0) {
        lin_lut_fill(lin_lut, kc, (int)threadIdx.x);
        __syncthreads();
    }
    constexpr int kWsPerTile = LANES / kGroup;
    static_assert(G::kWsWords <= kWsPerTile * Geometry<20>::kWsWords || L::kSlotsPerLane > 20, "workspace stride");
    uint32_t *wsA = ws_all + (size_t)(w.slot / kGroupsOfWave) * (8 * (size_t)kp.ws_words) + (w.g * LANES) * 4;
    uint32_t *wsB = wsA + 64 * 4;

    ChainState *st = chain_lds[group_in_block];
    if (w.gl < kSlots) { st[w.gl].phase = 2; st[w.gl].cand = -1; }
    wave_sync();
    bool exhausted = false;
    int my_bucket = 0;
    int bucket_first = 0;
    if (cq.leave_longest > 0) {
        int acc = 0;
        while (bucket_first < kBuckets && (acc += cq.bucket_count[bucket_first]) <= cq.leave_longest) bucket_first++;
        if (bucket_first >= kBuckets) bucket_first = 0;
    }
    bool second_set = false;
    constexpr bool one_set = !TWO_SETS;
    int idle_polls = 0;
    int rank_turn = 0, rank_cached = 0;
    __builtin_amdgcn_s_setprio(3);
#ifdef GACT_STAMPS
    unsigned long long stamp_acc[8] = {0, 0, 0, 0, 0, 0, 0, 0};
    const unsigned long long tl_start = __builtin_amdgcn_s_memrealtime();
    const unsigned long long tl_cyc0 = __builtin_amdgcn_s_memtime();
    unsigned long long tl_empty = 0;
#endif

    for (;;) {
        GACT_STAMP(t_a);
        PairTile pt;
        bool have[kSlots];
        int Tend_h[kSlots], tB_h[kSlots];
        int longest = 0;
#pragma unroll
        for (int h = 0; h < kSlots; h++) {
            ChainState s = st[h];
            TilePick pk;
            pk.have = false; pk.R = 0; pk.Q = 0; pk.reverse = false; pk.rp0 = 0; pk.qp0 = 0;
            for (int guard = 0; guard < 3 && !pk.have; guard++) {
                if (s.phase == 2) {
                    if (exhausted) break;
                    int cand = -1;
                    for (;;) {
                        const int *q_count = (TWO_SETS && second_set) ? cq.more_count : cq.bucket_count;
                        int *q_pop = (TWO_SETS && second_set) ? cq.more_pop : cq.bucket_pop;
                        const int *q_live = (TWO_SETS && second_set) ? cq.more_live : cq.live;
                        while (my_bucket < kBuckets) {
                            const int bkt = bucket_first + my_bucket - (bucket_first + my_bucket >= kBuckets ? kBuckets : 0);
                            const int cnt = q_count[bkt];
                            int idx = cnt;
                            if (w.gl == 0 && __hip_atomic_load(&q_pop[bkt], __ATOMIC_RELAXED, __HIP_MEMORY_SCOPE_AGENT) < cnt)
                                idx = atomicAdd(&q_pop[bkt], 1);
                            idx = __shfl(idx, 0, LANES);
                            if (idx < cnt) {
                                cand = q_live[(size_t)bkt * cq.live_stride + idx];
                                break;
                            }
                            my_bucket++;
                        }
                        if (cand >= 0 || second_set || one_set) break;
                        if (__hip_atomic_load(cq.more_flag, __ATOMIC_RELAXED, __HIP_MEMORY_SCOPE_AGENT) == 0) break;
                        __builtin_amdgcn_fence(__ATOMIC_ACQUIRE, "agent");
                        second_set = true;
                        my_bucket = 0;
                    }
                    if (cand < 0) {
                        if (second_set || one_set) {
                            exhausted = true;
#ifdef GACT_STAMPS
                            if (!tl_empty) tl_empty = __builtin_amdgcn_s_memrealtime();
#endif
                        }
                        break;
                    }
                    s = cq.states[cand];
                }
                pk = chain_pick(s, kp, same_file, out, w.gl == 0);
            }
            have[h] = pk.have;
            pt.R[h] = pk.R; pt.Q[h] = pk.Q; pt.reverse[h] = pk.reverse;
// ... 285 lines not shown
```

darwin-gpu_amd/csrc/gact_roles.hpp:

```cpp
#pragma once

#include "gact_lin.hpp"

namespace gact {

#ifndef GACT_ROLE_DP_WAVES
#define GACT_ROLE_DP_WAVES 10
#endif
constexpr int kRoleDp = GACT_ROLE_DP_WAVES;
constexpr int kRoleWalk = kRoleDp > 7 ? 2 : 1;
constexpr int kRoleThreads = 64 * (kRoleDp + kRoleWalk);
constexpr int kRoleBanks = 2;
constexpr int kRoleJobs = kRoleDp * 8;
constexpr int kRoleJobsPerWalker = kRoleJobs / kRoleWalk;
static_assert(kRoleDp % kRoleWalk == 0 && kRoleJobsPerWalker <= 64, "a walker wave serves whole DP waves, a lane per tile slot");
constexpr int kRoleCacheStride = 36;

struct WalkJob {
    uint32_t seq;
    uint32_t ws_off;
    int R, Q;
    int k0;
    int v0;
    int band_lim;
// ... 87 lines not shown
                go = (R >= 1) & (Q >= 1) & (early > 0) & (v != 0);
                fresh = true; active = true;
            }
        }
        if (!__any(active)) {
            if (*(__attribute__((address_space(3))) volatile const int *)dp_finished >= kRoleDp) break;
            if (idle < 64) __builtin_amdgcn_s_sleep(1); else __builtin_amdgcn_s_sleep(8);
            idle++;
            continue;
        }
        idle = 0;
        if (active && go) {
            tb_refill_oct<CW, QN, ROW>(ws_all, ws_off, scratch, l, c, k, rg);
            off0 = 4 * (-8 * rg.fbase[0] - 4 * rg.qbase0);
            off1 = 4 * (16 - 8 * rg.fbase[1] - 4 * (QN - 2));
            cur = fetch(l, c, k);
            bases();
        }
        (void)fresh;
#pragma unroll 1
        for (int m = 0; m < 8; m++) {
            if (!__any(go)) break;
            if (go) {
                const bool diag = cur == kM;
                const int sub = rcode == qcode ? v_match : v_mism;
                v -= diag ? sub : v_gap;
                nis -= cur != kD;
                njs -= cur != kI;
                const int p = imax(p0 + njs, 0);
                l = (int)(__umul24((uint32_t)p, kMagic) >> 16);
                c = p + __mul24(l, -CW);
                k = imax(kA + l + nis, 0);
                if (m == 7) {
                    redo = redo | ((band_lim >= 0) & ((unsigned)(nis - njs + band_lim) > (unsigned)(2 * band_lim)));
                } else {
                    cur = fetch(l, c, k);
                    bases();
                }
                go = !((diag && v == 0) || nis <= nlim_i || njs <= nlim_j || redo);
            }
        }
        if (active && !go) {
            WalkDone d;
            d.seq = seq; d.ref_steps = -nis; d.query_steps = -njs; d.dv = v0 - v; d.redo = redo ? 1 : 0;
            done[lane][bank].ref_steps = d.ref_steps; done[lane][bank].query_steps = d.query_steps;
            done[lane][bank].dv = d.dv; done[lane][bank].redo = d.redo;
            __builtin_amdgcn_fence(__ATOMIC_RELEASE, "workgroup");
            *(LdsFlag *)&done[lane][bank].seq = seq;
            if (bank) done_seq1 = seq; else done_seq0 = seq;
            active = false;
        }
    }
}

template <class L, bool TWO_SETS = false>
__global__ __launch_bounds__(kRoleThreads, 3) void extend_roles_kernel(
    KParams kp, P16Consts kc, SeqSetDev refs, SeqSetDev qfwd, SeqSetDev qrc,
    int same_file, gact_overlap *__restrict__ out, ChainQueues cq,
    uint32_t *__restrict__ ws_all)
{
    using G = typename L::G;
    constexpr int LANES = L::kLanes;
    static_assert(LANES == kGroup && L::kWalkFmt == 3 && L::kEndAligned, "the split linear-gap layout");
    constexpr int kGroupsOfWave = 64 / LANES;
    constexpr int kDpGroups = kRoleDp * kGroupsOfWave;
    constexpr int kStageWords = StageGeom<L::kSlotsPerLane, LANES>::kWords;
    constexpr int kSeg = StageGeom<L::kSlotsPerLane, LANES>::kSeg;
    static_assert(((kDpGroups * kRoleBanks * kStageWords) >> 15) == 0, "stage index fits WalkJob::where");
    __shared__ __attribute__((aligned(16))) uint8_t lds[kDpGroups * G::kGroupLds];
    __shared__ ChainState chain_lds[kDpGroups][kRoleBanks][kSlots];
    __shared__ __attribute__((aligned(16))) uint32_t stage_lds[kDpGroups][kRoleBanks][kStageWords];
    __shared__ WalkJob jobs[kRoleJobs][kRoleBanks];
    __shared__ WalkDone done[kRoleJobs][kRoleBanks];
    __shared__ __attribute__((aligned(16))) uint32_t cache_lds[kRoleJobs * kRoleCacheStride];
    __shared__ int dp_finished;
    __shared__ int bank_lds[kDpGroups][kRoleBanks][6];

    for (int n = threadIdx.x; n < kRoleJobs * kRoleBanks; n += kRoleThreads) {
        (&jobs[0][0])[n].seq = 0;
        (&done[0][0])[n].seq = 0;
    }
    if (threadIdx.x == 0) dp_finished = 0;
    uint32_t *const lin_lut = LinLutLds<L::kLutWords>::get();
    lin_lut_fill(lin_lut, kc, (int)threadIdx.x);
    __syncthreads();

    const int wave_in_block = threadIdx.x >> 6;
    if (wave_in_block >= kRoleDp) {
        __builtin_amdgcn_s_setprio(3);
        role_walker<L>(kp, ws_all, jobs, done, &stage_lds[0][0][0], cache_lds, &dp_finished);
        return;
    }

    WaveCtx w;
    {
        const int lane = threadIdx.x & 63;
        w.gl = lane & (LANES - 1);
        w.g = lane / LANES;
        w.slot = (blockIdx.x * kRoleDp + wave_in_block) * kGroupsOfWave + w.g;
        w.n_slots = gridDim.x * kRoleDp * kGroupsOfWave;
    }
    const int group_in_block = wave_in_block * kGroupsOfWave + w.g;
    uint8_t *ref8 = lds + group_in_block * G::kGroupLds;
    uint8_t *q8 = ref8 + G::kRefBytes;
    const uint16_t *ref16_lane = reinterpret_cast<const uint16_t *>(ref8) + (L::kRow0 - 1 - w.gl);
    uint32_t *ws_wave = ws_all + (size_t)(blockIdx.x * kRoleDp + wave_in_block) * (kRoleBanks * role_bank_words<L>());
    const int job_lane = wave_in_block * 8 + w.g * kSlots + (w.gl & 1);

    for (int b = 0; b < kRoleBanks; b++)
        if (w.gl < kSlots) { chain_lds[group_in_block][b][w.gl].phase = 2; chain_lds[group_in_block][b][w.gl].cand = -1; }
    wave_sync();
    bool exhausted = false;
    int my_bucket = 0;
    int bucket_first = 0;
    if (cq.leave_longest > 0) {
        int acc = 0;
        while (bucket_first < kBuckets && (acc += cq.bucket_count[bucket_first]) <= cq.leave_longest) bucket_first++;
        if (bucket_first >= kBuckets) bucket_first = 0;
    }
    bool second_set = false;
    constexpr bool one_set = !TWO_SETS;
    int idle_polls = 0;
    int rank_turn = 0, rank_cached = 0;
    int *bt = &bank_lds[group_in_block][0][0];
    if (w.gl == 0) {
        for (int n = 0; n < kRoleBanks * 6; n++) bt[n] = 0;
    }
    wave_sync();
    int bank = 0;
    __builtin_amdgcn_s_setprio(3);
#ifdef GACT_STAMPS
    unsigned long long stamp_acc[8] = {0, 0, 0, 0, 0, 0, 0, 0};
    const unsigned long long tl_start = __builtin_amdgcn_s_memrealtime();
    const unsigned long long tl_cyc0 = __builtin_amdgcn_s_memtime();
    unsigned long long tl_empty = 0;
#endif

    for (;;) {
        ChainState *st = chain_lds[group_in_block][bank];
        GACT_STAMP(t_w0);
        const int *bk = &bank_lds[group_in_block][bank][0];
        const uint32_t want = (uint32_t)__builtin_amdgcn_readfirstlane(bk[4]);
        if (want != 0) {
            typedef __attribute__((address_space(3))) volatile uint32_t LdsFlag;
            const int sv_R[kSlots] = {bk[0], bk[2]}, sv_Q[kSlots] = {bk[1], bk[3]};
            const bool mine = w.gl < kSlots && ((w.gl & 1) ? sv_R[1] : sv_R[0]) > 0;
            const unsigned long long wd0 = __builtin_amdgcn_s_memrealtime();
            for (;;) {
                const bool ok = !mine || *(LdsFlag *)&done[job_lane][bank].seq == want;
                if (__all(ok)) break;
                __builtin_amdgcn_s_sleep(2);
                if (__builtin_amdgcn_s_memrealtime() - wd0 > 200000000ull) {
                    if ((threadIdx.x & 63) == 0) atomicOr(cq.band_redos, 1 << 30);
                    break;
                }
            }
            __builtin_amdgcn_fence(__ATOMIC_ACQUIRE, "workgroup");
            int ref_steps = 0, query_steps = 0, nst = 0, redo = 0;
            ScoreWalk wk;
            wk.score = 0; wk.pend_gap = 0; wk.open_flag = 0; wk.have_left = 0; wk.left_first_gap = 0;
            if (mine) {
                const WalkDone d = done[job_lane][bank];
                wk.load(st[w.gl & 1]);
                wk.score += d.dv;
                ref_steps = d.ref_steps; query_steps = d.query_steps; nst = d.ref_steps + d.query_steps; redo = d.redo;
            }
#pragma unroll
// ... 185 lines not shown
```

darwin-gpu_amd/gact_amd/engine.py:

```python
import ctypes as C
import os
import subprocess

import numpy as np

_PKG = os.path.dirname(os.path.dirname(os.path.abspath(__file__)))
_ROOT = os.path.dirname(_PKG)
LIB_PATH = os.path.join(_PKG, "libgact_hip.so")
SOURCES = [os.path.join(_PKG, "csrc", f) for f in
           ("gact_engine.hip", "gact_kernels.hpp", "gact_device.hpp", "gact_chain.hpp", "gact_p16.hpp", "gact_p16s.hpp", "gact_lin.hpp",
            "gact_aff.hpp", "gact_roles.hpp", "gact_coop.hpp", "gact_policy.hpp", "gact_big.hpp", "gact_gather.hpp", "gact_chain_kernel.hpp", "gact_path.hpp", "gact_summary.hpp", "gact_select.hpp", "gact_cover.hpp", "gact_pileup.hpp",
            "dsoft_device.hpp", "dsoft_engine.hpp")] + \
          [os.path.join(_ROOT, "include", "gact_hip.h")]

SET_REF, SET_QUERY, SET_QUERY_RC = 0, 1, 2
STATE_Z, STATE_D, STATE_I, STATE_M = 0, 1, 2, 3

TILE_DTYPE = np.dtype([("ref_id", "<i4"), ("query_id", "<i4"), ("ref_off", "<i4"), ("query_off", "<i4"),
                       ("ref_len", "<i4"), ("query_len", "<i4"),
                       ("reverse", "u1"), ("first", "u1"), ("query_set", "u1"), ("pad", "u1")])
TILE_RESULT_DTYPE = np.dtype([(n, "<i4") for n in
                              ("score", "max_i", "max_j", "ref_steps", "query_steps", "n_states")])
CAND_DTYPE = np.dtype([(n, "<i4") for n in ("ref_id", "query_id", "ref_pos", "query_pos")])
OVERLAP_DTYPE = np.dtype([(n, "<i4") for n in
# ... 541 lines not shown
        if n_reads is None:
            n_reads = max(n_all - int(read_first), 0)
        self._pileup = None
        self._check(self.L.gact_hip_pileup_begin(self.h, int(read_first), int(n_reads)))
        offs = self._ref_offsets
        self._pileup = (int(n_reads), int(offs[int(read_first) + int(n_reads)] - offs[int(read_first)]))

    def pileup_add(self, sel=None, n=None, rc_from=0x7fffffff, same_file=True, slot=0):
        if sel is not None:
            sel = np.ascontiguousarray(sel, dtype=np.int32)
            n = len(sel)
        self._check(self.L.gact_hip_pileup_add(self.h, slot, int(n or 0), sel.ctypes.data if sel is not None else None,
                                               int(rc_from), int(same_file)))

    def pileup_finish(self, min_depth=3, counts=True, consensus=True):
        if self._pileup is None:
            raise GactHipError("gact_hip error -1: pileup_finish: no window is open (gact_hip_pileup_begin first)")
        n_reads, n_pos = self._pileup
        reads = np.zeros(n_reads, dtype=READ_PILEUP_DTYPE)
        cnt = np.zeros((n_pos, 8), dtype=np.uint32) if counts else None
        cons = np.zeros(n_pos, dtype=np.uint8) if consensus else None
        ptr = lambda a: a.ctypes.data if a is not None else None
        self._check(self.L.gact_hip_pileup_finish(self.h, int(min_depth), ptr(cnt), ptr(cons), ptr(reads)))
        return reads, cnt, cons

    def last_pileup_stats(self):
        st = PileupStats()
        self._check(self.L.gact_hip_last_pileup_stats(self.h, C.byref(st)))
        return {n: getattr(st, n) for n, _ in PileupStats._fields_}

    def register_output(self, out, slot=0):
        assert out.flags["C_CONTIGUOUS"] and out.flags["WRITEABLE"]
        self._check(self.L.gact_hip_register_output(self.h, slot, out.ctypes.data, out.nbytes))
        self._registered[slot] = out

    def unregister_output(self, slot=0):
        self._check(self.L.gact_hip_unregister_output(self.h, slot))
        self._registered.pop(slot, None)

    def sync(self, slot=0):
        self._check(self.L.gact_hip_sync(self.h, slot))

    def prepare(self, expected_candidates=0):
        if hasattr(self.L, "gact_hip_prepare"):
            self.L.gact_hip_prepare.argtypes = [C.c_void_p, C.c_int32]
            self.L.gact_hip_prepare.restype = C.c_int
            self._check(self.L.gact_hip_prepare(self.h, int(expected_candidates)))

    def set_option(self, name, value):
        if hasattr(self.L, "gact_hip_set_option"):
            self._check(self.L.gact_hip_set_option(self.h, name.encode(), int(value)))

    def dsoft_build(self, params=None):
        params = params or DsoftParams()
        info = DsoftInfo()
        self._check(self.L.gact_hip_dsoft_build(self.h, C.byref(params), C.byref(info)))
        return {n: getattr(info, n) for n, _ in DsoftInfo._fields_}

    def dsoft_query(self, first_query, n_queries, slot=0):
        nf, nr, ms = C.c_int32(), C.c_int32(), C.c_float()
        self._check(self.L.gact_hip_dsoft_query(self.h, slot, first_query, n_queries, C.byref(nf), C.byref(nr),
                                                C.byref(ms)))
        self._n_cands[slot] = nf.value + nr.value
        return nf.value, nr.value, float(ms.value)

    def candidates_download(self, n, slot=0):
        out = np.zeros(n, dtype=CAND_DTYPE)
        self._check(self.L.gact_hip_candidates_download(self.h, slot, n, out.ctypes.data))
        return out

    def last_kernel_ms(self, slot=0):
        ms = C.c_float()
        self._check(self.L.gact_hip_last_kernel_ms(self.h, slot, C.byref(ms)))
        return float(ms.value)

    def last_run_stats(self, slot=0):
        st = RunStats()
        self._check(self.L.gact_hip_last_run_stats(self.h, slot, C.byref(st)))
        if st.band_redos & (1 << 30):
            raise GactHipError("the role launch's watchdog fired: a DP wave went on without its walker's results (records are wrong)")
        return {"total_ms": st.total_ms, "seed_ms": st.seed_ms, "main_ms": st.main_ms,
                "packed16": bool(st.packed16), "layout": ("int32", "packed16-uniform", "packed16-split", "packed16-wide")[st.packed16],
                "seed_layout": "packed16" if st.seed_packed16 else "int32",
                "tagged_pointers": bool(st.tagged_pointers), "linear_gap": st.linear_gap == 1, "affine_drift": st.linear_gap == 2,
                "handed_off": st.handed_off, "seed_cells": st.seed_cells, "raw_candidates": st.raw_candidates,
                "band_redos": st.band_redos, "merged_callers": st.merged_callers, "overlapped_seeding": bool(st.overlapped_seeding),
                "critical_lane": bool(st.critical_lane), "role_waves": st.role_waves == 1, "coop_walks": st.role_waves == 2}

    def measure_valu_rate(self):
        v = C.c_double()
        self._check(self.L.gact_hip_measure_valu_rate(self.h, C.byref(v)))
        return float(v.value)

    def device_overlaps_ptr(self, slot=0):
        return self.L.gact_hip_device_overlaps(self.h, slot)

    def format_overlap(self, rec, ref_name, query_name):
        rec = np.ascontiguousarray(rec, dtype=OVERLAP_DTYPE)
        buf = C.create_string_buffer(512)
        n = self._check(self.L.gact_hip_format_overlap(rec.ctypes.data, ref_name.encode(), query_name.encode(),
                                                       buf, 512))
        return buf.raw[:n].decode()


def format_paf(rec, summary, query_name, query_len, ref_name, ref_len, cap=1024):
    L = load()
    rec = np.ascontiguousarray(rec, dtype=OVERLAP_DTYPE)
    summary = np.ascontiguousarray(summary, dtype=SUMMARY_DTYPE)
    buf = C.create_string_buffer(cap)
    n = L.gact_hip_format_paf(rec.ctypes.data, summary.ctypes.data, query_name.encode(), int(query_len), ref_name.encode(),
                              int(ref_len), buf, cap)
    if n < 0:
        raise GactHipError("gact_hip error %d: %s" % (n, L.gact_hip_last_error().decode()))
    return buf.raw[:min(n, cap - 1)].decode()


class Comm:

    LINE_DTYPE = np.dtype([(n, "<i4") for n in ("ref_id", "query_id", "ab", "ae", "bb", "be", "score", "comp_emitted")])

    def __init__(self, eng, rank, world, id_path, timeout_s=120):
        self.eng, self.rank, self.world = eng, rank, world
        self.h = C.c_void_p()
        eng._check(eng.L.gact_hip_comm_create(eng.h, rank, world, id_path.encode(), int(timeout_s), C.byref(self.h)))

    def gather_lines(self, n, slot=0, room=None):
        counts = np.zeros(self.world, dtype=np.int64)
        cap = int(room if room is not None else (n + 1) * self.world) if self.rank == 0 else 0
        lines = np.zeros(cap, dtype=self.LINE_DTYPE) if self.rank == 0 else None
        self.eng._check(self.eng.L.gact_hip_comm_gather_lines(self.h, slot, int(n), counts.ctypes.data,
                                                              lines.ctypes.data if lines is not None else None, cap))
        return counts, (lines[:int(counts.sum())] if lines is not None else None)

    def close(self):
        if self.h:
            self.eng.L.gact_hip_comm_destroy(self.h)
            self.h = C.c_void_p()


def queue_from_tile(result, states, first):
    n = int(result["n_states"])
    st = [int(x) for x in states[:n]]
    if first:
        return [int(result["score"]), int(result["max_i"]), int(result["max_j"])] + st
    return [int(result["score"])] + st
```

Measured before the change: 9211 GCUPS.

## Add column-drift linear-gap DP pass with gap folded into the LUT

Adds a new split linear-gap DP pass that keeps scores relative to a per-column drift rather than a per-row one. The gap penalty is folded into the substitution lookup table, and hand-written DPP sub/max sequences with SGPR operands do the cross-lane handoff. The default SplitLayoutLin now uses this pass. The old row-drift pass is kept as SplitLayoutLinRow and is used only when the match and gap scores would overflow the column-drift range. The aim is to cut VALU instructions per cell in the inner loop, at the cost of more inline-asm complexity, hand-placed s_nop hazards, and extra kernel instantiations.

```diff
diff --git a/darwin-gpu_amd/csrc/gact_coop.hpp b/darwin-gpu_amd/csrc/gact_coop.hpp
--- a/darwin-gpu_amd/csrc/gact_coop.hpp
+++ b/darwin-gpu_amd/csrc/gact_coop.hpp
@@ -166,7 +166,7 @@
     uint32_t *const lin_lut = LinLutLds<L::kLutWords>::get();
     for (int n = threadIdx.x; n < kCoopJobs; n += kBlockThreads) jstate[n] = 0;
     if (threadIdx.x == 0) walk_lock = 0;
-    lin_lut_fill(lin_lut, kc, (int)threadIdx.x);
+    lin_lut_fill_for_pass<L>(lin_lut, kc, (int)threadIdx.x);
     __syncthreads();
 
     const int wave_in_block = threadIdx.x >> 6;
diff --git a/darwin-gpu_amd/csrc/gact_engine.hip b/darwin-gpu_amd/csrc/gact_engine.hip
--- a/darwin-gpu_amd/csrc/gact_engine.hip
+++ b/darwin-gpu_amd/csrc/gact_engine.hip
@@ -385,6 +385,7 @@
     bool split = false;
     bool tagged = false;
     bool lin = false;
+    bool lin_row = false;
     bool aff = false;
     bool aff_seed = true;
     int wide = 0;
@@ -789,12 +790,23 @@
         }
         using gact::extend_p16_kernel;
         using RolesL = gact::SplitLayoutLin<7, 13>;
+        using RowL = gact::SplitLayoutLinRow<7, 13>;
+        using RowTeamL = gact::SplitLayoutLinRowTeam<7, 13>;
+        const bool lin_row = e->lin_row;
         auto launch_main = [&](pol::MainK k, bool two_sets, int blocks, hipStream_t stream, const gact::ChainQueues &q, uint32_t *ws) -> int {
             using M = pol::MainK;
             const dim3 g((unsigned)blocks), b256(gact::kBlockThreads), brole(gact::kRoleThreads);
 #define GACT_LAUNCH_MAIN(KERNEL, BLOCK) hipLaunchKernelGGL(KERNEL, g, BLOCK, 0, stream, kp, e->kc, d_rs, d_qf, d_qr, same_file, sl.overlaps.p, q, ws)
             if constexpr (C == 20) {
-                switch (k) {
+                if (lin_row) switch (k) {
+                case M::RolesLin: if (two_sets) GACT_LAUNCH_MAIN((gact::extend_roles_kernel<RowL, true>), brole); else GACT_LAUNCH_MAIN((gact::extend_roles_kernel<RowL, false>), brole); break;
+                case M::CoopLin: if (two_sets) GACT_LAUNCH_MAIN((gact::extend_coop_kernel<RowL, true>), b256); else GACT_LAUNCH_MAIN((gact::extend_coop_kernel<RowL, false>), b256); break;
+                case M::SplitLin: if (two_sets) GACT_LAUNCH_MAIN((extend_p16_kernel<RowL, false, true>), b256); else GACT_LAUNCH_MAIN((extend_p16_kernel<RowL, false>), b256); break;
+                case M::SplitLinTeam: GACT_LAUNCH_MAIN((extend_p16_kernel<RowTeamL, false>), b256); break;
+                default: break;
+                }
+                const bool row_done = lin_row && (k == M::RolesLin || k == M::CoopLin || k == M::SplitLin || k == M::SplitLinTeam);
+                if (!row_done) switch (k) {
                 case M::RolesLin: if (two_sets) GACT_LAUNCH_MAIN((gact::extend_roles_kernel<RolesL, true>), brole); else GACT_LAUNCH_MAIN((gact::extend_roles_kernel<RolesL, false>), brole); break;
                 case M::CoopLin: if (two_sets) GACT_LAUNCH_MAIN((gact::extend_coop_kernel<RolesL, true>), b256); else GACT_LAUNCH_MAIN((gact::extend_coop_kernel<RolesL, false>), b256); break;
                 case M::SplitLin: if (two_sets) GACT_LAUNCH_MAIN((extend_p16_kernel<gact::SplitLayoutLin<7, 13>, false, true>), b256); else GACT_LAUNCH_MAIN((extend_p16_kernel<gact::SplitLayoutLin<7, 13>, false>), b256); break;
@@ -997,10 +1009,14 @@
     int a = 0;
     HIP_TRY(hipOccupancyMaxActiveBlocksPerMultiprocessor(&a, gact::extend_p16_kernel<gact::SplitLayoutLin<7, 13>, false>,
                                                          gact::kBlockThreads, 0));
-    int b = a;
+    int b = a, c = a, d = a;
     HIP_TRY(hipOccupancyMaxActiveBlocksPerMultiprocessor(&b, gact::extend_p16_kernel<gact::SplitLayoutLinTeam<7, 13>, false>,
                                                          gact::kBlockThreads, 0));
-    *out = std::max(1, std::min(a, b));
+    HIP_TRY(hipOccupancyMaxActiveBlocksPerMultiprocessor(&c, gact::extend_p16_kernel<gact::SplitLayoutLinRow<7, 13>, false>,
+                                                         gact::kBlockThreads, 0));
+    HIP_TRY(hipOccupancyMaxActiveBlocksPerMultiprocessor(&d, gact::extend_p16_kernel<gact::SplitLayoutLinRowTeam<7, 13>, false>,
+                                                         gact::kBlockThreads, 0));
+    *out = std::max(1, std::min(std::min(a, b), std::min(c, d)));
     return 0;
 }
 
@@ -1096,6 +1112,7 @@
                 opt_env("no_tagged") == nullptr;
     e->lin = e->tagged && gact::p16_lin_ok(p->tile_size, p->match, p->mismatch, p->gap_open, p->gap_extend) &&
              opt_env("no_lin") == nullptr;
+    e->lin_row = e->lin && !gact::lin_col_drift_ok(p->match, p->gap_extend);
     e->aff = e->tagged && e->split && !e->lin && gact::p16_aff_ok(p->tile_size, p->match, p->mismatch, p->gap_open, p->gap_extend) &&
              opt_env("no_aff") == nullptr;
     e->aff_seed = opt_env("no_aff_seed") == nullptr;
@@ -1220,13 +1237,16 @@
     e->role_grid_blocks = 0;
     if (e->lin && e->split && e->C == 20) {
         using RL = gact::SplitLayoutLin<7, 13>;
-        int rb = 0, rb2 = 0;
+        using RowL = gact::SplitLayoutLinRow<7, 13>;
+        int rb = 0, rb2 = 0, rb3 = 0, rb4 = 0;
         if (hipOccupancyMaxActiveBlocksPerMultiprocessor(&rb, gact::extend_roles_kernel<RL, false>, gact::kRoleThreads, 0) != hipSuccess ||
-            hipOccupancyMaxActiveBlocksPerMultiprocessor(&rb2, gact::extend_roles_kernel<RL, true>, gact::kRoleThreads, 0) != hipSuccess) {
+            hipOccupancyMaxActiveBlocksPerMultiprocessor(&rb2, gact::extend_roles_kernel<RL, true>, gact::kRoleThreads, 0) != hipSuccess ||
+            hipOccupancyMaxActiveBlocksPerMultiprocessor(&rb3, gact::extend_roles_kernel<RowL, false>, gact::kRoleThreads, 0) != hipSuccess ||
+            hipOccupancyMaxActiveBlocksPerMultiprocessor(&rb4, gact::extend_roles_kernel<RowL, true>, gact::kRoleThreads, 0) != hipSuccess) {
             delete e;
             return fail(GACT_HIP_EDEVICE, "hipOccupancyMaxActiveBlocksPerMultiprocessor failed");
         }
-        e->role_grid_blocks = std::max(1, std::min(rb, rb2)) * e->prop.multiProcessorCount;
+        e->role_grid_blocks = std::max(1, std::min(std::min(rb, rb2), std::min(rb3, rb4))) * e->prop.multiProcessorCount;
         if (const char *v = opt_env("role_blocks")) e->role_grid_blocks = std::max(1, std::min(atoi(v), e->role_grid_blocks));
     }
     e->roles = e->roles && e->role_grid_blocks > 0;
@@ -2210,7 +2230,7 @@
         st->packed16 = rec->two_phase ? (rec->wide ? 3 : e->split ? 2 : 1) : 0;
         st->seed_packed16 = (rec->two_phase && e->seed16) ? 1 : 0;
         st->tagged_pointers = (rec->two_phase && e->tagged) ? 1 : 0;
-        st->linear_gap = (rec->two_phase && rec->lin) ? 1 : (rec->two_phase && rec->aff) ? 2 : 0;
+        st->linear_gap = (rec->two_phase && rec->lin) ? ((e->lin_row && !rec->wide) ? 3 : 1) : (rec->two_phase && rec->aff) ? 2 : 0;
         st->raw_candidates = rec->routed_raw;
         if (rec->two_phase) {
             HIP_TRY(hipEventElapsedTime(&st->seed_ms, rec->ev0, rec->ev_mid));
@@ -2241,7 +2261,7 @@
     st->packed16 = sl.two_phase ? (sl.wide ? 3 : e->split ? 2 : 1) : 0;
     st->seed_packed16 = (sl.two_phase && e->seed16) ? 1 : 0;
     st->tagged_pointers = (sl.two_phase && e->tagged) ? 1 : 0;
-    st->linear_gap = (sl.two_phase && sl.lin) ? 1 : (sl.two_phase && sl.aff) ? 2 : 0;
+    st->linear_gap = (sl.two_phase && sl.lin) ? ((e->lin_row && !sl.wide) ? 3 : 1) : (sl.two_phase && sl.aff) ? 2 : 0;
     st->raw_candidates = sl.routed_raw;
     if (sl.two_phase) {
         HIP_TRY(hipEventElapsedTime(&st->seed_ms, sl.ev0, sl.ev_mid));
@@ -2300,20 +2320,24 @@
             for (hipStream_t st : {sl.stream, sl.aux_stream}) {
                 hipLaunchKernelGGL((gact::seed_p16_kernel<20, false, 1>), dim3(1), dim3(gact::kBlockThreads), 0, st, e->kp, e->kc, d, d, d,
                                    sl.cands.p, 0, 0, 0, 0, sl.overlaps.p, q, sl.d_ws);
-                hipLaunchKernelGGL((gact::extend_p16_kernel<gact::SplitLayoutLin<7, 13>, false>), dim3(1), dim3(gact::kBlockThreads), 0, st, e->kp,
-                                   e->kc, d, d, d, 0, sl.overlaps.p, q, sl.d_ws);
-                hipLaunchKernelGGL((gact::extend_p16_kernel<gact::SplitLayoutLin<7, 13>, false, true>), dim3(1), dim3(gact::kBlockThreads), 0, st,
-                                   e->kp, e->kc, d, d, d, 0, sl.overlaps.p, q2, sl.d_ws);
-                hipLaunchKernelGGL((gact::extend_coop_kernel<gact::SplitLayoutLin<7, 13>, false>), dim3(1), dim3(gact::kBlockThreads), 0, st,
-                                   e->kp, e->kc, d, d, d, 0, sl.overlaps.p, q, sl.d_ws);
-                hipLaunchKernelGGL((gact::extend_coop_kernel<gact::SplitLayoutLin<7, 13>, true>), dim3(1), dim3(gact::kBlockThreads), 0, st,
-                                   e->kp, e->kc, d, d, d, 0, sl.overlaps.p, q2, sl.d_ws);
-                if (e->role_grid_blocks > 0) {
-                    hipLaunchKernelGGL((gact::extend_roles_kernel<gact::SplitLayoutLin<7, 13>, false>), dim3(1), dim3(gact::kRoleThreads), 0, st,
+                auto warm = [&](auto layout) {
+                    using WL = decltype(layout);
+                    hipLaunchKernelGGL((gact::extend_p16_kernel<WL, false>), dim3(1), dim3(gact::kBlockThreads), 0, st, e->kp,
+                                       e->kc, d, d, d, 0, sl.overlaps.p, q, sl.d_ws);
+                    hipLaunchKernelGGL((gact::extend_p16_kernel<WL, false, true>), dim3(1), dim3(gact::kBlockThreads), 0, st,
+                                       e->kp, e->kc, d, d, d, 0, sl.overlaps.p, q2, sl.d_ws);
+                    hipLaunchKernelGGL((gact::extend_coop_kernel<WL, false>), dim3(1), dim3(gact::kBlockThreads), 0, st,
                                        e->kp, e->kc, d, d, d, 0, sl.overlaps.p, q, sl.d_ws);
-                    hipLaunchKernelGGL((gact::extend_roles_kernel<gact::SplitLayoutLin<7, 13>, true>), dim3(1), dim3(gact::kRoleThreads), 0, st,
+                    hipLaunchKernelGGL((gact::extend_coop_kernel<WL, true>), dim3(1), dim3(gact::kBlockThreads), 0, st,
                                        e->kp, e->kc, d, d, d, 0, sl.overlaps.p, q2, sl.d_ws);
-                }
+                    if (e->role_grid_blocks > 0) {
+                        hipLaunchKernelGGL((gact::extend_roles_kernel<WL, false>), dim3(1), dim3(gact::kRoleThreads), 0, st,
+                                           e->kp, e->kc, d, d, d, 0, sl.overlaps.p, q, sl.d_ws);
+                        hipLaunchKernelGGL((gact::extend_roles_kernel<WL, true>), dim3(1), dim3(gact::kRoleThreads), 0, st,
+                                           e->kp, e->kc, d, d, d, 0, sl.overlaps.p, q2, sl.d_ws);
+                    }
+                };
+                if (e->lin_row) warm(gact::SplitLayoutLinRow<7, 13>{}); else warm(gact::SplitLayoutLin<7, 13>{});
                 HIP_TRY(hipGetLastError());
             }
             HIP_TRY(hipStreamSynchronize(sl.stream));
diff --git a/darwin-gpu_amd/csrc/gact_lin.hpp b/darwin-gpu_amd/csrc/gact_lin.hpp
--- a/darwin-gpu_amd/csrc/gact_lin.hpp
+++ b/darwin-gpu_amd/csrc/gact_lin.hpp
@@ -27,14 +27,16 @@
 #ifndef GACT_LIN_BUILTINS
 #define GACT_LIN_BUILTINS 0
 #endif
+__host__ inline bool lin_col_drift_ok(int match, int ext) { return match - 2 * ext <= 63; }
+constexpr bool kLinSplitBuiltins = true;
 typedef short LinS2 __attribute__((ext_vector_type(2)));
+template <bool BUILTIN = GACT_LIN_BUILTINS>
 __device__ __forceinline__ uint32_t lin_max(uint32_t a, uint32_t b)
 {
-#if GACT_LIN_BUILTINS
-    return __builtin_bit_cast(uint32_t, __builtin_elementwise_max(__builtin_bit_cast(LinS2, a), __builtin_bit_cast(LinS2, b)));
-#else
-    return pk_max(a, b);
-#endif
+    if constexpr (BUILTIN)
+        return __builtin_bit_cast(uint32_t, __builtin_elementwise_max(__builtin_bit_cast(LinS2, a), __builtin_bit_cast(LinS2, b)));
+    else
+        return pk_max(a, b);
 }
 __device__ __forceinline__ uint32_t lin_sub(uint32_t a, uint32_t b)
 {
@@ -56,15 +58,54 @@
     asm("v_pk_maximum3_f16 %0, %1, %2, %3" : "=v"(r) : "v"(a), "v"(b), "v"(c));
     return r;
 }
+__device__ __forceinline__ uint32_t pk_max3f_s(uint32_t a, uint32_t s_b, uint32_t c)
+{
+    uint32_t r;
+    asm("v_pk_maximum3_f16 %0, %1, %2, %3" : "=v"(r) : "v"(a), "s"(s_b), "v"(c));
+    return r;
+}
+__device__ __forceinline__ uint32_t pk_max_sgpr(uint32_t a, uint32_t s_b)
+{
+    uint32_t r;
+    asm("v_pk_max_i16 %0, %1, %2" : "=v"(r) : "v"(a), "s"(s_b));
+    return r;
+}
+#define GACT_DPP_SHR1 " row_shr:1 row_mask:0xf bank_mask:0xf"
+#define GACT_DPP_ROR1 " row_ror:1 row_mask:0xf bank_mask:0xf"
+__device__ __forceinline__ uint32_t lin_hand_shr1(uint32_t h, uint32_t v_k, uint32_t s_old)
+{
+    uint32_t r;
+    asm("v_mov_b32 %0, %3\n\ts_nop 0\n\tv_sub_u32_dpp %0, %1, %2" GACT_DPP_SHR1 : "=&v"(r) : "v"(h), "v"(v_k), "s"(s_old));
+    return r;
+}
+__device__ __forceinline__ uint32_t lin_hand_ror1_shr1(uint32_t h1, uint32_t v_k1, uint32_t h2, uint32_t v_k2)
+{
+    uint32_t r;
+    asm("s_nop 1\n\tv_sub_u32_dpp %0, %1, %2" GACT_DPP_ROR1 "\n\tv_sub_u32_dpp %0, %3, %4" GACT_DPP_SHR1
+        : "=&v"(r) : "v"(h1), "v"(v_k1), "v"(h2), "v"(v_k2));
+    return r;
+}
+__device__ __forceinline__ uint32_t lin_hand_scaled_ror1(uint32_t h1, uint32_t v_c)
+{
+    uint32_t r;
+    asm("v_pk_mad_u16 %0, %1, 4, %2 op_sel_hi:[1,0,1]\n\ts_nop 1\n\tv_mov_b32_dpp %0, %0" GACT_DPP_ROR1 : "=&v"(r) : "v"(h1), "v"(v_c));
+    return r;
+}
+__device__ __forceinline__ uint32_t lin_hand_shr1_over(uint32_t first, uint32_t h2, uint32_t v_k2)
+{
+    asm("s_nop 1\n\tv_sub_u32_dpp %0, %1, %2" GACT_DPP_SHR1 : "+v"(first) : "v"(h2), "v"(v_k2));
+    return first;
+}
+template <bool BUILTIN = GACT_LIN_BUILTINS>
 __device__ __forceinline__ uint32_t andn_or(uint32_t a, uint32_t b, uint32_t c)
 {
-#if GACT_LIN_BUILTINS
-    return __builtin_amdgcn_bitop3_b32(a, b, c, 0xba);
-#else
-    uint32_t r;
-    asm("v_bitop3_b32 %0, %1, %2, %3 bitop3:0xba" : "=v"(r) : "v"(a), "v"(b), "v"(c));
-    return r;
-#endif
+    if constexpr (BUILTIN)
+        return __builtin_amdgcn_bitop3_b32(a, b, c, 0xba);
+    else {
+        uint32_t r;
+        asm("v_bitop3_b32 %0, %1, %2, %3 bitop3:0xba" : "=v"(r) : "v"(a), "v"(b), "v"(c));
+        return r;
+    }
 }
 __device__ __forceinline__ uint32_t pk_ashr2(uint32_t a)
 {
@@ -413,6 +454,288 @@
     }
     return tagged ? pk_ashr2(lin_sub(H2 | kc.c3, Z24)) : lin_sub(H2, Z2);
 }
+
+template <int C1, int C2>
+__device__ __forceinline__ uint32_t dp_pass_lin_split_col(const P16Consts &kc, const int gl,
+                                                      const uint16_t *__restrict__ ref16,
+                                                      const uint32_t (&qb)[C1 + C2],
+                                                      const int T_end, const int tB,
+                                                      uint32_t *__restrict__ wsA, uint32_t *__restrict__ wsB,
+                                                      const int band, const bool fullA, const bool fullB,
+                                                      const uint32_t *lut_lds)
+{
+    constexpr int CT = C1 + C2;
+    constexpr int NW = LinWords<C2>::kWords, QD = LinWords<C2>::kUint4;
+    constexpr int LAG = kGroup;
+    const int g = (int)(int16_t)(kc.ext & 0xffffu);
+    const uint32_t gs = kc.next, g4s = kc.next4;
+    const uint32_t k1v = vconst((uint32_t)(C1 - 1) * kc.next),
+                   k2v = vconst((uint32_t)(C2 - 1) * kc.next);
+    uint32_t c3v = 0, onev = 0, c2v = 0,
+             k24v = 0,
+             k12v = 0;
+    const uint32_t psel = sconst_here(kLinPairSel);
+    constexpr int NWIN = C2 + 1;
+    uint32_t W[NWIN], T[C2];
+#pragma unroll
+    for (int k = 0; k < NWIN; k++) W[k] = pk2(lin_base(g) + (k - 1) * (-g));
+#pragma unroll
+    for (int c = 0; c < C2; c++) T[c] = 0;
+    auto bump = [](uint32_t &z, const uint32_t by) { asm("s_add_u32 %0, %0, %1" : "+s"(z) : "s"(by) : "scc"); };
+    auto advance = [&](const int nW, const bool tagged_too) {
+#pragma unroll
+        for (int k = 0; k < NWIN; k++) if (k < nW) { if (tagged_too) bump(W[k], gs); else W[k] += gs; }
+        if (tagged_too) {
+#pragma unroll
+            for (int c = 0; c < C2; c++) bump(T[c], g4s);
+        }
+    };
+    uint32_t G[CT];
+    uint32_t acc[2 * NW];
+    uint32_t grp[2 * (C2 / 2)], odd = 0;
+#pragma unroll
+    for (int c = 0; c < CT; c++) G[c] = W[(c < C1 ? c : c - C1) + 1];
+#pragma unroll
+    for (int c = 0; c < 2 * NW; c++) acc[c] = 0;
+    uint32_t H1 = W[C1], H2 = W[C2];
+    uint32_t Hdiag1 = W[0], Hdiag2 = W[0];
+
+    typedef __attribute__((address_space(3))) const uint8_t LdsByte;
+    typedef __attribute__((address_space(3))) const uint32_t LdsWord;
+    LdsByte *const lut_plain = (LdsByte *)lut_lds, *const lut_tagged = (LdsByte *)(lut_lds + 1);
+    auto row = [](LdsByte *table, uint32_t stream_byte) { return *(LdsWord *)(table + stream_byte); };
+    LdsByte *rp = (LdsByte *)(ref16 + (1 - LAG));
+    uint32_t rb1 = row(lut_plain, rp[2 * LAG]), rb1b = row(lut_plain, rp[2 * LAG + 1]);
+    uint32_t rb2 = row(lut_plain, rp[0]), rb2b = row(lut_plain, rp[1]);
+    rp += 2;
+
+#define GACT_SB() __builtin_amdgcn_sched_barrier(0)
+    uint32_t sb1 = 0, sb1b = 0, sb2 = 0, sb2b = 0;
+    auto ask_bytes = [&](const bool r1, const bool r2) {
+        if (r2) { sb2 = rp[0]; sb2b = rp[1]; }
+        if (r1) { sb1 = rp[2 * LAG]; sb1b = rp[2 * LAG + 1]; }
+        rp += 2;
+    };
+    auto ask_rows = [&](const bool r1, const bool r2, const bool tag2) {
+        if (r1) { rb1 = row(lut_plain, sb1); rb1b = row(lut_plain, sb1b); }
+        if (r2) { rb2 = row(tag2 ? lut_tagged : lut_plain, sb2); rb2b = row(tag2 ? lut_tagged : lut_plain, sb2b); }
+    };
+    auto upper_all = [&](uint32_t (&U)[CT], const bool tag2) {
+        uint32_t P[CT];
+#pragma unroll
+        for (int c = 0; c < CT; c++) P[c] = __builtin_amdgcn_perm(c < C1 ? rb1b : rb2b, c < C1 ? rb1 : rb2, qb[c]);
+        GACT_SB();
+#pragma unroll
+        for (int c = 0; c < CT; c++) U[c] = (c == 0 ? Hdiag1 : c == C1 ? Hdiag2 : G[c - 1]) + P[c];
+        ask_rows(true, true, tag2);
+        GACT_SB();
+        if (GACT_LIN_MAX3) {
+#pragma unroll
+            for (int c = 0; c < CT; c++)
+                U[c] = pk_max3f_s(U[c], c < C1 ? W[c + 1] : tag2 ? T[c - C1] : W[c - C1 + 1], G[c]);
+        } else {
+#pragma unroll
+            for (int c = 0; c < CT; c++) U[c] = pk_max_sgpr(U[c], c < C1 ? W[c + 1] : tag2 ? T[c - C1] : W[c - C1 + 1]);
+            GACT_SB();
+#pragma unroll
+            for (int c = 0; c < CT; c++) U[c] = lin_max<kLinSplitBuiltins>(U[c], G[c]);
+        }
+        GACT_SB();
+    };
+
+    auto step = [&]() {
+        ask_bytes(true, true);
+        advance(NWIN, false);
+        const uint32_t Hl1 = lin_hand_shr1(H1, k1v, W[0]);
+        const uint32_t Hl2 = lin_hand_ror1_shr1(H1, k1v, H2, k2v);
+        uint32_t U[CT];
+        upper_all(U, false);
+        Hdiag1 = Hl1; Hdiag2 = Hl2;
+        uint32_t Ha = Hl1, Hb = Hl2;
+        static_assert(C2 >= C1, "region 2 is the longer chain");
+#pragma unroll
+        for (int c = 0; c < C1; c++) {
+            G[c] = lin_max<kLinSplitBuiltins>(U[c], Ha); G[C1 + c] = lin_max<kLinSplitBuiltins>(U[C1 + c], Hb);
+            GACT_SB();
+            Ha = G[c]; Hb = G[C1 + c];
+        }
+#pragma unroll
+        for (int c = 2 * C1; c < CT; c++) { G[c] = lin_max<kLinSplitBuiltins>(U[c], Hb); Hb = G[c]; }
+        H1 = Ha; H2 = Hb;
+    };
+    auto step_r1 = [&]() {
+        ask_bytes(true, false);
+        advance(C1 + 1, false);
+        const uint32_t Hl1 = lin_hand_shr1(H1, k1v, W[0]);
+        uint32_t P[C1], U[C1];
+#pragma unroll
+        for (int c = 0; c < C1; c++) P[c] = __builtin_amdgcn_perm(rb1b, rb1, qb[c]);
+        GACT_SB();
+#pragma unroll
+        for (int c = 0; c < C1; c++) U[c] = (c == 0 ? Hdiag1 : G[c - 1]) + P[c];
+        ask_rows(true, false, false);
+        GACT_SB();
+#pragma unroll
+        for (int c = 0; c < C1; c++) U[c] = GACT_LIN_MAX3 ? pk_max3f_s(U[c], W[c + 1], G[c]) : lin_max<kLinSplitBuiltins>(pk_max_sgpr(U[c], W[c + 1]), G[c]);
+        GACT_SB();
+        Hdiag1 = Hl1;
+        uint32_t Ha = Hl1;
+#pragma unroll
+        for (int c = 0; c < C1; c++) { G[c] = lin_max<kLinSplitBuiltins>(U[c], Ha); Ha = G[c]; }
+        H1 = Ha;
+    };
+
+    static_assert(C2 >= 3 && (C2 & 1), "the last pair is filed while the unpaired slot is computed");
+    auto file_group = [&](const int S, const int c, const uint32_t x) {
+        uint32_t &r = grp[c - 2 + (S >> 2)];
+        r = (S & 3) ? pk_shl_add4(r, x) : x;
+    };
+    auto step_tagged = [&](auto pos) {
+        constexpr int S = decltype(pos)::value;
+        constexpr bool blk = S != kLinTail;
+        ask_bytes(true, true);
+        advance(C1 + 1, true);
+        const uint32_t Hl1 = lin_hand_shr1(H1, k1v, W[0]);
+        const uint32_t Hl2 = lin_hand_shr1_over(lin_hand_scaled_ror1(H1, k12v), H2, k24v);
+        uint32_t U[CT];
+        upper_all(U, true);
+        Hdiag1 = Hl1; Hdiag2 = Hl2;
+        uint32_t Ha = Hl1, Hb = Hl2;
+        uint32_t tprev = 0, Hq = 0, x = 0;
+#pragma unroll
+        for (int c = 0; c < C2; c++) {
+            const bool both = c < C1;
+            const bool filed = blk && c >= 2 && !(c & 1);
+            const uint32_t Db = Hb - onev;
+            if (filed) x &= kLinPairMask;
+            GACT_SB();
+            const uint32_t Hp = lin_max<kLinSplitBuiltins>(U[C1 + c], Db);
+            if (both) { G[c] = lin_max<kLinSplitBuiltins>(U[c], Ha); Ha = G[c]; }
+            if (!blk && c > 0) acc[c - 1] = pk_shl_add4(acc[c - 1], tprev);
+            if (filed) file_group(S, c, x);
+            GACT_SB();
+            G[C1 + c] = andn_or<kLinSplitBuiltins>(Hp, c3v, c2v);
+            if (!blk || c == C2 - 1) tprev = Hp & c3v;
+            else if (c & 1) x = __builtin_amdgcn_perm(Hp, Hq, psel);
+            else Hq = Hp;
+            GACT_SB();
+            Hb = G[C1 + c];
+        }
+        if (!blk) acc[C2 - 1] = pk_shl_add4(acc[C2 - 1], tprev);
+        else odd = S ? pk_shl_add4(odd, tprev) : tprev;
+        H1 = Ha; H2 = Hb;
+    };
+    auto step_tagged_r2 = [&](auto pos) {
+        constexpr int S = decltype(pos)::value;
+        constexpr bool blk = S != kLinTail;
+        ask_bytes(false, true);
+        advance(0, true);
+        const uint32_t Hl2 = lin_hand_shr1_over(lin_hand_scaled_ror1(H1, k12v), H2, k24v);
+        uint32_t P[C2], U[C2];
+#pragma unroll
+        for (int c = 0; c < C2; c++) P[c] = __builtin_amdgcn_perm(rb2b, rb2, qb[C1 + c]);
+        GACT_SB();
+#pragma unroll
+        for (int c = 0; c < C2; c++) U[c] = (c == 0 ? Hdiag2 : G[C1 + c - 1]) + P[c];
+        ask_rows(false, true, true);
+        GACT_SB();
+#pragma unroll
+        for (int c = 0; c < C2; c++) U[c] = GACT_LIN_MAX3 ? pk_max3f_s(U[c], T[c], G[C1 + c]) : lin_max<kLinSplitBuiltins>(pk_max_sgpr(U[c], T[c]), G[C1 + c]);
+        GACT_SB();
+        Hdiag2 = Hl2;
+        uint32_t Hb = Hl2;
+        uint32_t tprev = 0, Hq = 0, x = 0;
+#pragma unroll
+        for (int c = 0; c < C2; c++) {
+            const bool filed = blk && c >= 2 && !(c & 1);
+            const uint32_t Db = Hb - onev;
+            if (filed) x &= kLinPairMask;
+            GACT_SB();
+            const uint32_t Hp = lin_max<kLinSplitBuiltins>(U[c], Db);
+            if (!blk && c > 0) acc[c - 1] = pk_shl_add4(acc[c - 1], tprev);
+            if (filed) file_group(S, c, x);
+            GACT_SB();
+            G[C1 + c] = andn_or<kLinSplitBuiltins>(Hp, c3v, c2v);
+            if (!blk || c == C2 - 1) tprev = Hp & c3v;
+            else if (c & 1) x = __builtin_amdgcn_perm(Hp, Hq, psel);
+            else Hq = Hp;
+            GACT_SB();
+            Hb = G[C1 + c];
+        }
+        if (!blk) acc[C2 - 1] = pk_shl_add4(acc[C2 - 1], tprev);
+        else odd = S ? pk_shl_add4(odd, tprev) : tprev;
+        H2 = Hb;
+    };
+#define GACT_LIN_BLOCK8(f) do { f(LinPos<0>{}); f(LinPos<1>{}); f(LinPos<2>{}); f(LinPos<3>{}); \
+                                f(LinPos<4>{}); f(LinPos<5>{}); f(LinPos<6>{}); f(LinPos<7>{}); } while (0)
+#undef GACT_SB
+    auto enter_tagged = [&]() {
+        c3v = vconst(kc.c3); onev = vconst(kc.one); c2v = vconst(kc.tag2);
+        k24v = vconst((uint32_t)(C2 - 1) * kc.next4);
+        k12v = vconst(pk2(2 + 4 * (C1 - 1) * g));
+#pragma unroll
+        for (int c = C1; c < CT; c++) G[c] = pk_mad4v(G[c], c2v);
+        H2 = pk_mad4v(H2, c2v);
+        Hdiag2 = pk_mad4v(Hdiag2, c2v);
+#pragma unroll
+        for (int c = 0; c < C2; c++) T[c] = (W[c + 1] << 2) + kc.c3;
+        rb2 = row(lut_tagged, rp[-2]); rb2b = row(lut_tagged, rp[-1]);
+    };
+
+    int t = 1;
+    for (const int tP = imin(LAG, imin(tB - 1, T_end)); t <= tP; t++) step_r1();
+    if (t > 1) {
+#pragma unroll
+        for (int k = C1 + 1; k < NWIN; k++) W[k] = W[k - 1] + gs;
+#pragma unroll
+        for (int c = C1; c < CT; c++) G[c] = W[c - C1 + 1];
+        H2 = W[C2]; Hdiag2 = W[0];
+        rb2 = row(lut_plain, rp[-2]); rb2b = row(lut_plain, rp[-1]);
+    }
+    const int tU = imin(tB - 1, T_end);
+    for (; t + 1 <= tU; t += 2) { step(); step(); }
+    if (t <= tU) { step(); t++; }
+    const bool tagged = t <= T_end;
+    if (tagged) enter_tagged();
+    uint4 *qA = reinterpret_cast<uint4 *>(wsA) + gl;
+    uint4 *qB = reinterpret_cast<uint4 *>(wsB) + gl;
+    LinBand bd;
+    {
+        const int q1 = (band >> 16) - 1, b = band & 0xffff;
+        const int u_lo = kGroup - 1 - (gl & ~q1), u_hi = kGroup - 1 - (gl | q1);
+        LinBand lo_, hi_;
+        lin_band_range(lo_, 0, T_end, u_lo, C2 * u_lo, C2 * u_lo + C2 - 1, b, fullA);
+        lin_band_range(hi_, 0, T_end, u_hi, C2 * u_hi, C2 * u_hi + C2 - 1, b, fullA);
+        bd.lo[0] = bd.lo[1] = lo_.lo[0]; bd.hi[0] = bd.hi[1] = hi_.hi[0];
+        bd.full[0] = fullA | (b <= 0); bd.full[1] = fullB | (b <= 0);
+    }
+    int k = 0;
+    while (t + 7 <= T_end && t <= T_end - LAG) {
+        GACT_LIN_BLOCK8(step_tagged);
+        t += 8; k += 8;
+        lin_flush_groups<C2>(grp, odd, qA, qB, bd.store(0, t - 8, t - 1), bd.store(1, t - 8, t - 1));
+        qA += QD * kWsRow;
+        qB += QD * kWsRow;
+    }
+    while (t + 7 <= T_end) {
+        GACT_LIN_BLOCK8(step_tagged_r2);
+        t += 8; k += 8;
+        lin_flush_groups<C2>(grp, odd, qA, qB, bd.store(0, t - 8, t - 1), bd.store(1, t - 8, t - 1));
+        qA += QD * kWsRow;
+        qB += QD * kWsRow;
+    }
+#undef GACT_LIN_BLOCK8
+    for (; t <= T_end - LAG; t++, k++) step_tagged(LinPos<kLinTail>{});
+    for (; t <= T_end; t++, k++) step_tagged_r2(LinPos<kLinTail>{});
+    if (k & 7) {
+        const int sh = 2 * (8 - (k & 7));
+        lin_flush<NW, kGroup>(acc, qA, qB, [sh](uint32_t w) { return ((w & 0xffffu) << sh & 0xffffu) | ((w >> 16) << sh << 16); },
+                              bd.store(0, t - (k & 7), t - 1), bd.store(1, t - (k & 7), t - 1));
+    }
+    return tagged ? pk_ashr2(lin_sub(H2 | kc.c3, T[C2 - 1])) : lin_sub(H2, W[C2]);
+}
+#undef GACT_DPP_SHR1
+#undef GACT_DPP_ROR1
 
 template <int C, int LANES, bool AMAX>
 __device__ __forceinline__ uint32_t dp_pass_lin(const P16Consts &kc, const int gl,
@@ -666,6 +989,7 @@
     static constexpr int kWalkSpan = GACT_WALK_SPAN;
     static constexpr bool kEndAligned = true;
     static constexpr int kLutWords = kLinLutWords;
+    static constexpr bool kColDrift = true;
     using Base = SplitLayout<C1, C2, true>;
     template <bool RAW>
     __device__ static void load(const SeqSetDev &rs, const SeqSetDev &qf, const SeqSetDev &qr,
@@ -680,9 +1004,24 @@
                                     int T_end, int tB, uint32_t *wsA, uint32_t *wsB, const PairTile &pt)
     {
         static_assert(!RAW, "the linear-gap pass reads 2-bit sets");
+        return dp_pass_lin_split_col<C1, C2>(kc, gl, ref16, qb, T_end, tB, wsA, wsB, pt.band, pt.full[0], pt.full[1], pt.lut);
+    }
+    __device__ static int fin_lane(int Q) { (void)Q; return kGroup - 1; }
+};
+
+template <int C1, int C2> struct SplitLayoutLinRow : SplitLayoutLin<C1, C2> {
+    static constexpr bool kColDrift = false;
+    template <bool RAW>
+    __device__ static uint32_t pass(const P16Consts &kc, int gl, const uint16_t *ref16, const uint32_t (&qb)[C1 + C2],
+                                    int T_end, int tB, uint32_t *wsA, uint32_t *wsB, const PairTile &pt)
+    {
+        static_assert(!RAW, "the linear-gap pass reads 2-bit sets");
         return dp_pass_lin_split<C1, C2>(kc, gl, ref16, qb, T_end, tB, wsA, wsB, pt.band, pt.full[0], pt.full[1], pt.lut);
     }
-    __device__ static int fin_lane(int Q) { (void)Q; return kGroup - 1; }
+};
+
+template <int C1, int C2> struct SplitLayoutLinRowTeam : SplitLayoutLinRow<C1, C2> {
+    static constexpr bool kTeamWalk = true;
 };
 
 template <int C1, int C2> struct SplitLayoutLinTeam : SplitLayoutLin<C1, C2> {
diff --git a/darwin-gpu_amd/csrc/gact_p16.hpp b/darwin-gpu_amd/csrc/gact_p16.hpp
--- a/darwin-gpu_amd/csrc/gact_p16.hpp
+++ b/darwin-gpu_amd/csrc/gact_p16.hpp
@@ -462,6 +462,21 @@
         lut[tid] = (b < kLinPadRow ? base >> b : 0u) + ((tid & 1) ? 0x01010101u : 0u);
     }
 }
+__device__ __forceinline__ void lin_lut_fill_col(uint32_t *lut, const P16Consts &kc, const int tid)
+{
+    if (tid < kLinLutWords) {
+        const uint32_t b = 8u * ((uint32_t)tid >> 1), base = (tid & 1) ? kc.dsub4 : kc.dsub;
+        const uint32_t gap = (((tid & 1) ? kc.next4 : kc.next) & 0xffu) * 0x01010101u;
+        lut[tid] = (b < kLinPadRow ? (base >> b) + gap : 0u) + ((tid & 1) ? 0x01010101u : 0u);
+    }
+}
+template <class L, class = void> struct lin_col_drift { static constexpr bool value = false; };
+template <class L> struct lin_col_drift<L, std::void_t<decltype(L::kColDrift)>> { static constexpr bool value = L::kColDrift; };
+template <class L>
+__device__ __forceinline__ void lin_lut_fill_for_pass(uint32_t *lut, const P16Consts &kc, const int tid)
+{
+    if constexpr (lin_col_drift<L>::value) lin_lut_fill_col(lut, kc, tid); else lin_lut_fill(lut, kc, tid);
+}
 template <int N> struct LinLutLds {
     __device__ __forceinline__ static uint32_t *get() { __shared__ __attribute__((aligned(8))) uint32_t words[N]; return words; }
 };
@@ -712,7 +727,7 @@
     const uint16_t *ref16_lane = reinterpret_cast<const uint16_t *>(ref8) + (L::kRow0 - 1 - w.gl);
     uint32_t *const lin_lut = LinLutLds<lin_lut_words<L>::value>::get();
     if constexpr (lin_lut_words<L>::value > 0) {
-        lin_lut_fill(lin_lut, kc, (int)threadIdx.x);
+        lin_lut_fill_for_pass<L>(lin_lut, kc, (int)threadIdx.x);
         __syncthreads();
     }
     constexpr int kWsPerTile = LANES / kGroup;
diff --git a/darwin-gpu_amd/csrc/gact_roles.hpp b/darwin-gpu_amd/csrc/gact_roles.hpp
--- a/darwin-gpu_amd/csrc/gact_roles.hpp
+++ b/darwin-gpu_amd/csrc/gact_roles.hpp
@@ -193,7 +193,7 @@
     }
     if (threadIdx.x == 0) dp_finished = 0;
     uint32_t *const lin_lut = LinLutLds<L::kLutWords>::get();
-    lin_lut_fill(lin_lut, kc, (int)threadIdx.x);
+    lin_lut_fill_for_pass<L>(lin_lut, kc, (int)threadIdx.x);
     __syncthreads();
 
     const int wave_in_block = threadIdx.x >> 6;
diff --git a/darwin-gpu_amd/gact_amd/engine.py b/darwin-gpu_amd/gact_amd/engine.py
--- a/darwin-gpu_amd/gact_amd/engine.py
+++ b/darwin-gpu_amd/gact_amd/engine.py
@@ -647,7 +647,7 @@
         return {"total_ms": st.total_ms, "seed_ms": st.seed_ms, "main_ms": st.main_ms,
                 "packed16": bool(st.packed16), "layout": ("int32", "packed16-uniform", "packed16-split", "packed16-wide")[st.packed16],
                 "seed_layout": "packed16" if st.seed_packed16 else "int32",
-                "tagged_pointers": bool(st.tagged_pointers), "linear_gap": st.linear_gap == 1, "affine_drift": st.linear_gap == 2,
+                "tagged_pointers": bool(st.tagged_pointers), "linear_gap": st.linear_gap in (1, 3), "lin_row_drift": st.linear_gap == 3, "affine_drift": st.linear_gap == 2,
                 "handed_off": st.handed_off, "seed_cells": st.seed_cells, "raw_candidates": st.raw_candidates,
                 "band_redos": st.band_redos, "merged_callers": st.merged_callers, "overlapped_seeding": bool(st.overlapped_seeding),
                 "critical_lane": bool(st.critical_lane), "role_waves": st.role_waves == 1, "coop_walks": st.role_waves == 2}
```

Result: faster. 9422 GCUPS, median of 6 (+2.3%).
